# pangenome/povu

Measured on AMD Instinct MI355X. Metric: edges/sec decomposed (flubble+PVST), higher is better.
Workload: dtype u32

## Files before the change

include/povu_hip.h:

```cpp
#ifndef POVU_HIP_H
#define POVU_HIP_H

#include <stddef.h>
#include <stdint.h>

#ifdef __cplusplus
extern "C" {
#endif

#define POVU_HIP_NIL 0xFFFFFFFFu
#define POVU_SIDE_L 0
#define POVU_SIDE_R 1
#define POVU_TIP_NONE 0
#define POVU_TIP_L 1
#define POVU_TIP_R 2

typedef struct povu_hip_ctx povu_hip_ctx;
typedef struct povu_hip_forest povu_hip_forest;

int povu_hip_device_count(void);

povu_hip_ctx *povu_hip_create(int device, char *err, size_t errlen);
void povu_hip_destroy(povu_hip_ctx *ctx);
int povu_hip_release_workspace(povu_hip_ctx *ctx);
// ... 320 lines not shown
char *povu_hip_pvst_format(uint32_t n_pvst, const uint32_t *a_id, const uint32_t *z_id, const uint8_t *a_or,
			   const uint8_t *z_or, const uint32_t *parent, size_t *len);
char *povu_hip_pvst_format_fam(uint32_t n_pvst, const uint32_t *a_id, const uint32_t *z_id, const uint8_t *a_or,
			       const uint8_t *z_or, const uint32_t *parent, const uint8_t *fam, size_t *len);
void povu_hip_buffer_free(void *p);

typedef struct {
	uint32_t n;
	char *type;
	uint32_t *file_id;
	uint32_t *a_id, *z_id;
	uint8_t *a_or, *z_or;
	uint8_t *route;
	uint32_t *parent;
	uint32_t *height;
} povu_pvst_doc;
povu_pvst_doc *povu_pvst_parse(const char *text, size_t len, char *err, size_t errlen);

int povu_hip_gfa_write(const char *path, uint32_t n_vtx, const uint32_t *vid, uint32_t n_links, const uint32_t *v1,
		       const uint8_t *s1, const uint32_t *v2, const uint8_t *s2, char *err, size_t errlen);
void povu_pvst_doc_free(povu_pvst_doc *doc);

typedef struct {
	povu_hip_call_refs refs;
	uint32_t n_paths;
	const uint32_t *slot_of_path;
	const char *const *sample;
} povu_hip_call_names;
povu_hip_call_names *povu_hip_call_names_make(uint32_t n_paths, const char *const *path_name, uint32_t n_prefixes,
					      const char *const *prefix, char *err, size_t errlen);
void povu_hip_call_names_free(povu_hip_call_names *n);
int povu_hip_sites_add_tree(povu_hip_sites *s, uint32_t tree, uint32_t n, const uint32_t *id1, const uint32_t *id2,
			    const uint8_t *or1, const uint8_t *or2, const uint32_t *parent, const uint8_t *family);
povu_hip_sites *povu_hip_sites_of_docs(const povu_pvst_doc *const *docs, uint32_t n);
povu_hip_sites *povu_hip_forest_sites(const povu_hip_forest *f);
void povu_hip_sites_free(povu_hip_sites *s);
char *povu_hip_calls_vcf(const povu_hip_calls *c, const povu_hip_sites *sites, const povu_hip_call_names *names,
			 const char *const *path_name, const char *date, const char *only_prefix, uint32_t threads, size_t *len);
char *povu_hip_calls_vcf_profile(const povu_hip_calls *c, const povu_hip_sites *sites, const povu_hip_call_names *names,
				 const char *const *path_name, const char *date, const char *only_prefix, uint32_t threads, uint32_t profile,
				 size_t *len);
char *povu_hip_calls_vcf_rest(const povu_hip_calls *c, const povu_hip_sites *sites, const povu_hip_call_names *names,
			      const char *const *path_name, const char *date, const char *const *prefix, uint32_t n_prefixes, uint32_t threads,
			      uint32_t profile, size_t *len);

typedef struct {
	char name[48];
	double ms;
	uint32_t launches;
} povu_hip_stage_time;
int povu_hip_last_stage_times(const povu_hip_ctx *ctx, povu_hip_stage_time *out, int max);
uint32_t povu_hip_last_seq_redo(const povu_hip_ctx *ctx);
int povu_hip_last_black_only_classes(const povu_hip_ctx *ctx);
int povu_hip_last_laminar_check_ran(const povu_hip_ctx *ctx);
int povu_hip_last_crossings(povu_hip_ctx *ctx, uint32_t out[2]);
uint64_t povu_hip_last_links_processed(const povu_hip_ctx *ctx);

int povu_hip_debug_components(povu_hip_ctx *ctx, uint32_t *comp_of, uint32_t *local_idx);
int povu_hip_debug_tree(povu_hip_ctx *ctx, uint32_t comp, uint32_t *n_tree, uint32_t *gid, uint8_t *typ,
			uint32_t *par, uint32_t *cls);
int povu_hip_debug_edge_ids(povu_hip_ctx *ctx, uint32_t comp, uint32_t *n_tree, uint32_t *tree_edge_id);
int povu_hip_debug_stack(povu_hip_ctx *ctx, uint32_t comp, uint32_t *n, uint32_t *tree_vtx, uint32_t *cls,
			 uint32_t *next_seen);

#define POVU_HIP_SCAN_SUM 0
#define POVU_HIP_SCAN_MAX 1
#define POVU_HIP_SCAN_U64 2
#define POVU_HIP_SCAN_U8 3
#define POVU_HIP_SCAN_DIFF 4
#define POVU_HIP_SCAN_XOR_PAIR 5
#define POVU_HIP_SCAN_XOR_U128 6
#define POVU_HIP_SCAN_IN_PLACE 0x100
#define POVU_HIP_SCAN_N_DEV 0x200
int povu_hip_debug_scan(povu_hip_ctx *ctx, int op, const uint32_t *in, uint32_t *out, size_t n, const uint32_t *in2,
			uint32_t *out2, size_t n2);
int povu_hip_debug_sort(povu_hip_ctx *ctx, const uint32_t *keys, const uint32_t *vals, size_t n, unsigned bits,
			uint32_t *keys_out, uint32_t *vals_out);
int povu_hip_debug_compact(povu_hip_ctx *ctx, const uint8_t *flags, size_t n, uint32_t *out, uint32_t *count);
int povu_hip_debug_totals(povu_hip_ctx *ctx, const uint32_t *a, const uint32_t *b, size_t n, uint64_t tot[2]);
#define POVU_HIP_SEG_MIN 0
#define POVU_HIP_SEG_FIRST_LESS 1
#define POVU_HIP_SEG_LAST_LESS 2
int povu_hip_debug_segtree(povu_hip_ctx *ctx, const uint32_t *val, size_t n, const uint32_t *queries, size_t nq, uint32_t *out,
			   uint32_t *tree, uint32_t *P);
int povu_hip_debug_bitrank(povu_hip_ctx *ctx, const uint8_t *flags, size_t n, const uint32_t *pos, size_t nq, uint32_t *rank,
			   uint32_t *test, uint32_t *records);
int povu_hip_debug_append(povu_hip_ctx *ctx, const uint8_t *flags, size_t n, uint32_t *list, uint32_t *count);
int povu_hip_debug_list_rank(povu_hip_ctx *ctx, uint32_t n, const uint32_t *next, const uint8_t *w, const uint32_t *heads,
			     uint32_t nh, int mode, uint32_t bits, uint32_t *ra, uint32_t *rb);
double povu_hip_debug_scan_time(povu_hip_ctx *ctx, size_t n, int reps, int op);

uint64_t povu_hip_workspace_estimate(uint32_t n_vtx, uint32_t n_links, uint32_t n_components);
int povu_hip_workspace_breakdown(uint32_t n_vtx, uint32_t n_links, uint32_t n_components, uint64_t out[7]);
int povu_hip_prewarm(povu_hip_ctx *ctx, uint32_t n_vtx, uint32_t n_links, char *err, size_t errlen);
uint64_t povu_hip_leaf_workspace_estimate(uint32_t n_vtx, uint32_t n_components);

const char *povu_hip_version(void);

#ifdef __cplusplus
}
#endif
#endif
```

povu_amd/csrc/hip/common.hpp:

```cpp
#pragma once
#include <hip/hip_runtime.h>

#include <algorithm>
#include <cstdint>
#include <cstdio>
#include <cstring>
#include <stdexcept>
#include <string>
#include <vector>

#define POVU_NIL 0xFFFFFFFFu

__device__ __forceinline__ uint4 load4_unaligned(const unsigned *__restrict__ p)
{
	typedef unsigned v4a __attribute__((ext_vector_type(4), aligned(4)));
	const v4a v = *reinterpret_cast<const v4a *>(p);
	return make_uint4(v.x, v.y, v.z, v.w);
}

#ifdef POVU_XCD_SWIZZLE
__device__ __forceinline__ unsigned povu_xcd_bid()
{
	const unsigned nwg = gridDim.x, q = nwg >> 3, r = nwg & 7u, x = blockIdx.x & 7u, i = blockIdx.x >> 3;
	return (x < r ? x * (q + 1) : r * (q + 1) + (x - r) * q) + i;
// ... 220 lines not shown
		hipEvent_t a, b;
		uint32_t launches;
	};
	std::vector<Rec> recs;
	std::vector<hipEvent_t> pool;
	size_t pool_used = 0;
	hipStream_t stream = nullptr;
	bool enabled = true;
	hipEvent_t get()
	{
		if (pool_used == pool.size()) {
			hipEvent_t e;
			HIP_CHECK(hipEventCreate(&e));
			pool.push_back(e);
		}
		return pool[pool_used++];
	}
	void reset()
	{
		recs.clear();
		pool_used = 0;
	}
	void begin(const char *name)
	{
		if (!enabled)
			return;
		Rec r{name, get(), get(), 0};
		HIP_CHECK(hipEventRecord(r.a, stream));
		recs.push_back(r);
	}
	void end(uint32_t launches)
	{
		if (!enabled)
			return;
		recs.back().launches = launches;
		HIP_CHECK(hipEventRecord(recs.back().b, stream));
	}
	~StageTimer()
	{
		for (auto e : pool)
			(void)hipEventDestroy(e);
	}
};

void scan_exclusive_u32(const uint32_t *in, uint32_t *out, size_t n, void *tmp, size_t tmp_bytes, hipStream_t s);
void scan_exclusive_u32_pair(const uint32_t *in0, uint32_t *out0, size_t n0, const uint32_t *in1, uint32_t *out1, size_t n1,
			     void *tmp, size_t tmp_bytes, hipStream_t s);
void scan_exclusive_xor_u32_pair(const uint32_t *in0, uint32_t *out0, const uint32_t *in1, uint32_t *out1, size_t n, void *tmp,
				 size_t tmp_bytes, hipStream_t s);
void scan_exclusive_u8(const uint8_t *in0, uint32_t *out0, size_t n0, const uint8_t *in1, uint32_t *out1, size_t n1, void *tmp,
		       size_t tmp_bytes, hipStream_t s);
void scan_exclusive_diff_u32(const uint32_t *in, const uint32_t *sub, uint32_t *out, size_t n, void *tmp, size_t tmp_bytes,
			     hipStream_t s);
void scan_exclusive_xor_u128(const ulonglong2 *in, ulonglong2 *out, size_t n, void *tmp, size_t tmp_bytes, hipStream_t s,
			     const uint32_t *n_dev = nullptr);
size_t scan_tmp_bytes(size_t n);
void scan_exclusive_u64(const uint64_t *in, uint64_t *out, size_t n, uint64_t *tmp, hipStream_t s);
size_t scan_exclusive_u64_tmp(size_t n);
__device__ __forceinline__ uint32_t bitrank(const uint4 *__restrict__ rec, uint32_t x)
{
	const uint4 r = rec[x >> 6];
	const unsigned long long bits = (unsigned long long)r.x | ((unsigned long long)r.y << 32);
	return r.z + (uint32_t)__popcll(bits & ((1ull << (x & 63u)) - 1ull));
}
__device__ __forceinline__ bool bitrank_test(const uint4 *__restrict__ rec, uint32_t x)
{
	const uint4 r = rec[x >> 6];
	return (((x & 32u) ? r.y : r.x) >> (x & 31u)) & 1u;
}
struct StackComp {
	const uint4 *rec;
	const uint32_t *list;
	__device__ __forceinline__ uint32_t operator()(uint32_t i) const { return list[bitrank(rec, i + 1) - 1u]; }
};
__device__ __forceinline__ unsigned long long spread4(unsigned long long x)
{
	x &= 0xFFFFull;
	x = (x | (x << 24)) & 0x000000FF000000FFull;
	x = (x | (x << 12)) & 0x000F000F000F000Full;
	x = (x | (x << 6)) & 0x0303030303030303ull;
	x = (x | (x << 3)) & 0x1111111111111111ull;
	return x;
}
__device__ __forceinline__ void bitrank_store_wave(uint4 *__restrict__ rec, uint32_t f, bool in_range)
{
	const uint32_t lane = threadIdx.x & 63u;
	const unsigned long long m0 = __ballot(f & 1u), m1 = __ballot(f & 2u), m2 = __ballot(f & 4u), m3 = __ballot(f & 8u);
	if (lane < 4 && in_range) {
		const unsigned sh = 16u * lane;
		const unsigned long long w = spread4(m0 >> sh) | (spread4(m1 >> sh) << 1) | (spread4(m2 >> sh) << 2) | (spread4(m3 >> sh) << 3);
		rec[lane] = make_uint4((uint32_t)w, (uint32_t)(w >> 32), 0u, 0u);
	}
}
void bitrank_build(uint4 *rec, size_t n_rec, uint32_t *tmp_counts, void *scan_tmp, size_t scan_tmp_bytes, hipStream_t s);

static constexpr uint32_t LIST_ITER = 16, LIST_TPB = 256, LIST_SPAN = LIST_TPB * 4 * LIST_ITER;
__device__ __forceinline__ void append_in_order(unsigned long long fw, uint32_t B0, uint32_t *__restrict__ list, uint32_t *__restrict__ n_list)
{
	__shared__ uint32_t tot[LIST_ITER * (LIST_TPB / 64)], base_sh;
	const uint32_t lane = threadIdx.x & 63u, wave = threadIdx.x >> 6;
	const unsigned long long lt = (1ull << lane) - 1ull;
#pragma unroll
	for (uint32_t it = 0; it < LIST_ITER; it++) {
		const uint32_t f = (uint32_t)(fw >> (4 * it)) & 15u;
		const uint32_t t = (uint32_t)(__popcll(__ballot(f & 1u)) + __popcll(__ballot(f & 2u)) + __popcll(__ballot(f & 4u)) + __popcll(__ballot(f & 8u)));
		if (lane == 0)
// ... 54 lines not shown
```

povu_amd/csrc/hip/context.hpp:

```cpp
#pragma once
#include "../../../include/povu_hip.h"

#include "forest_wire.hpp"
#include "graph_kernels.hpp"
#include "leaf_kernels.hpp"
#include "par_kernels.hpp"
#include "seq_kernels.hpp"
#include "sub_kernels.hpp"
#include "tree_kernels.hpp"

#include <map>
#include <memory>
#include <mutex>
#include <numeric>
#include <string>

using namespace povu_hip;

struct PinnedPool {
	struct Block {
		void *p;
		size_t cap;
		int seg;
	};
// ... 144 lines not shown
		if (!q) {
			b.pool = pool;
			b.p = pool->get(block_bytes_for(total) + meta_bytes(meta_reserve), b.cap, &b.seg);
		}
		b.bytes = layout(b.p, total, &b);
		blocks.push_back(std::move(b));
		return blocks.back();
	}
	void release_blocks()
	{
		for (auto &b : blocks)
			if (b.p && b.pool)
				b.pool->put(b.p, b.cap, b.seg);
		blocks.clear();
	}
	~povu_hip_forest()
	{
		std::call_once(ready_once, [this] { wait_arrays(); });
		if (ev0)
			(void)hipEventDestroy(ev0);
		if (ev1)
			(void)hipEventDestroy(ev1);
		for (hipEvent_t e : more_events)
			(void)hipEventDestroy(e);
		release_blocks();
		if (xblk && pool)
			pool->put(xblk, xblk_cap, xblk_seg);
	}
	struct Tree : forest_wire::TreeRecord {
		int blk = 0;
	};
	std::vector<Tree> trees;
	std::vector<uint64_t> hairpins;
	void *xblk = nullptr;
	size_t xblk_cap = 0;
	int xblk_seg = -1;
	const void *walk_ctx = nullptr;
	uint64_t walk_gen = 0;
};

struct PassPlan {
	uint32_t rank = 0, world = 1;
	bool hairpins = false, all_seq = false, seq_tree = false, par_tree = true, leaf_sub = false, all_sub = false;
	bool sorted_adj = false, force_redo = false, redo_odd = false;
	bool big_class_dfs = false, sparse_splitters = false, all_vertex_classes = false, check_laminar = false;
	bool timed = true, overlap_tail = false, heaviest_first = false;
};

struct LastPass {
	bool valid = false;
	PassPlan plan;
	uint32_t C = 0, seq_redo = 0;
	bool mixed = false, redo_pvst_only = false, stack_export_pending = false;
};

struct povu_hip_ctx {
	int device = 0;
	hipStream_t stream = nullptr;
	SideStream side;
	ResidentGraph g;
	Arena ws_sub;
	size_t ws_sub_hint = 0;
	Arena ws, ws_b, ws2, ws_seq, ws_leaf, ws_walk, upload_tmp;
	HostScratch host;
	std::shared_ptr<PinnedPool> pool = std::make_shared<PinnedPool>();
	StageTimer timer;
	std::vector<povu_hip_stage_time> last_times;
	uint64_t last_links = 0;
	CompState cs{};
	SeqWs sw{};
	ParWs pw{};
	TreeWs tw{};
	LastPass last;
	std::vector<uint32_t> shard_comp_ids;
	uint32_t shard_total_components = 0;
	Arena shard_buf;
	Arena graph_arena;
	hipEvent_t tail_done = nullptr;
	SideStream walk_side;
	bool tail_pending = false;
	void wait_tail()
	{
		if (tail_pending) {
			(void)hipEventSynchronize(tail_done);
			tail_pending = false;
		}
	}
	void quiesce()
	{
		if (tail_pending) {
			(void)hipStreamSynchronize(stream);
			wait_tail();
		}
	}
	Arena wk_ws, wk_out;
	Arena paths_buf;
	uint32_t *path_steps = nullptr;
	uint64_t *path_off = nullptr;
	uint32_t n_paths = 0;
	uint64_t n_path_steps = 0, paths_gen = 0;
	bool paths_valid = false;
	Arena tr_ws, tr_task, tr_trav, tr_steps;
	Arena seq_buf, cl_ws, cl_slot, cl_rec, cl_spell, cl_bytes;
	Arena iv_ws, iv_heads, iv_rows;
	Arena nm_ws;
	Arena pr_ws, pr_slab, pr_rows;
// ... 67 lines not shown
```

povu_amd/csrc/hip/debug_hooks.hip:

```cpp
#include "context.hpp"
#include "segtree.hpp"

#include <algorithm>
#include <numeric>

using namespace povu_hip;

namespace
{
constexpr size_t DBG_GUARD = 256;
constexpr int DBG_GUARD_BYTE = 0xC5, DBG_POISON_BYTE = 0xA7;
constexpr int DBG_RC_GUARD = 5;
struct DbgOut {
	size_t bytes = 0;
	int fill = DBG_GUARD_BYTE;
	bool on = true;
	char *base = nullptr;
	size_t span = 0;
	template <class T>
	T *data() const { return reinterpret_cast<T *>(base + DBG_GUARD); }
	void declare(Spans &take, hipStream_t s)
	{
		if (!on)
			return;
// ... 12 lines not shown
	{
		take(bytes, p);
		if (take.ar && bytes)
			HIP_CHECK(hipMemsetAsync(p, DBG_POISON_BYTE, bytes, s));
	}
};
template <class T>
struct DbgIn {
	const T *host = nullptr;
	size_t n = 0;
	bool on = true;
	const T *dev = nullptr;
	void declare(Spans &take, hipStream_t s)
	{
		T *d = nullptr;
		if (on)
			take(n + 16, d);
		if (take.ar && on && n)
			HIP_CHECK(copy_async(d, host, n * sizeof(T), hipMemcpyHostToDevice, s));
		dev = d;
	}
};
template <class... B>
void dbg_carve(Arena &ar, hipStream_t s, B &...buf)
{
	carve(ar, [&](Spans &take) { (buf.declare(take, s), ...); });
}
bool dbg_all_guard(const void *host, size_t from, size_t to)
{
	const unsigned char *p = static_cast<const unsigned char *>(host);
	for (size_t i = from; i < to; i++)
		if (p[i] != (unsigned char)DBG_GUARD_BYTE)
			return false;
	return true;
}
bool dbg_guards_intact(const DbgOut &o, hipStream_t s)
{
	if (!o.base)
		return true;
	const size_t back = o.span - DBG_GUARD - o.bytes;
	std::vector<unsigned char> h(DBG_GUARD + back);
	HIP_CHECK(copy_async(h.data(), o.base, DBG_GUARD, hipMemcpyDeviceToHost, s));
	HIP_CHECK(copy_async(h.data() + DBG_GUARD, o.base + DBG_GUARD + o.bytes, back, hipMemcpyDeviceToHost, s));
	HIP_CHECK(hipStreamSynchronize(s));
	return dbg_all_guard(h.data(), 0, h.size());
}
}

extern "C" int povu_hip_debug_scan(povu_hip_ctx *ctx, int op, const uint32_t *in, uint32_t *out, size_t n, const uint32_t *in2,
				   uint32_t *out2, size_t n2)
{
	const int kind = op & 0xFF;
	const bool in_place = (op & POVU_HIP_SCAN_IN_PLACE) != 0, with_len = (op & POVU_HIP_SCAN_N_DEV) != 0;
	if (!ctx || kind > POVU_HIP_SCAN_XOR_U128 || (op & ~(0xFF | POVU_HIP_SCAN_IN_PLACE | POVU_HIP_SCAN_N_DEV)))
		return 1;
	if (kind == POVU_HIP_SCAN_U8) {
		if ((n && (!in || !out)) || (in2 && n2 && !out2))
			return 1;
	} else if (!in || !out || (in2 && !out2 && kind != POVU_HIP_SCAN_DIFF)) {
		return 1;
	}
	if ((in_place && (kind > POVU_HIP_SCAN_U64 || in2)) || (with_len && kind != POVU_HIP_SCAN_XOR_U128) ||
	    ((kind == POVU_HIP_SCAN_DIFF || kind == POVU_HIP_SCAN_XOR_PAIR) && !in2))
		return 1;
	try {
		HIP_CHECK(hipSetDevice(ctx->device));
		hipStream_t s = ctx->stream;
		const size_t e_in = kind == POVU_HIP_SCAN_U8 ? 1 : kind == POVU_HIP_SCAN_U64 ? 8 : kind == POVU_HIP_SCAN_XOR_U128 ? 16 : 4;
		const size_t e_out = kind == POVU_HIP_SCAN_U64 ? 8 : kind == POVU_HIP_SCAN_XOR_U128 ? 16 : 4;
		const bool pair = in2 && (kind == POVU_HIP_SCAN_SUM || kind == POVU_HIP_SCAN_U8 || kind == POVU_HIP_SCAN_XOR_PAIR);
		const bool second_in = pair || kind == POVU_HIP_SCAN_DIFF;
		const size_t m = !second_in ? 0 : (kind == POVU_HIP_SCAN_SUM || kind == POVU_HIP_SCAN_U8) ? n2 : n;
		const size_t tb = kind == POVU_HIP_SCAN_U64 ? scan_exclusive_u64_tmp(n) * 8 : scan_tmp_bytes(std::max(n, m));
		const uint32_t len = (uint32_t)n2;
		Arena ar;
		DbgOut o1{n * e_out}, o2{m * e_out, DBG_GUARD_BYTE, pair};
		DbgScratch scr{tb};
		DbgIn<char> i1{reinterpret_cast<const char *>(in), n * e_in, !in_place}, i2{reinterpret_cast<const char *>(in2), m * e_in, second_in};
		DbgIn<uint32_t> ilen{&len, 1, with_len};
		dbg_carve(ar, s, o1, o2, scr, i1, i2, ilen);
		if (in_place)
			HIP_CHECK(copy_async(o1.data<char>(), in, n * e_in, hipMemcpyHostToDevice, s));
		if (with_len)
			HIP_CHECK(hipStreamSynchronize(s));
		const char *di = in_place ? o1.data<char>() : i1.dev, *di2 = i2.dev;
		const uint32_t *w1 = reinterpret_cast<const uint32_t *>(di), *w2 = reinterpret_cast<const uint32_t *>(di2);
		void *tmp = scr.p;
		switch (kind) {
		case POVU_HIP_SCAN_SUM:
			if (pair)
				scan_exclusive_u32_pair(w1, o1.data<uint32_t>(), n, w2, o2.data<uint32_t>(), m, tmp, tb, s);
			else
				scan_exclusive_u32(w1, o1.data<uint32_t>(), n, tmp, tb, s);
			break;
		case POVU_HIP_SCAN_MAX: scan_exclusive_max_u32(w1, o1.data<uint32_t>(), n, tmp, tb, s); break;
		case POVU_HIP_SCAN_U64:
			scan_exclusive_u64(reinterpret_cast<const uint64_t *>(di), o1.data<uint64_t>(), n, static_cast<uint64_t *>(tmp), s);
			break;
		case POVU_HIP_SCAN_U8:
			scan_exclusive_u8(reinterpret_cast<const uint8_t *>(di), o1.data<uint32_t>(), n,
					  pair ? reinterpret_cast<const uint8_t *>(di2) : nullptr, pair ? o2.data<uint32_t>() : nullptr, m, tmp, tb, s);
			break;
		case POVU_HIP_SCAN_DIFF: scan_exclusive_diff_u32(w1, w2, o1.data<uint32_t>(), n, tmp, tb, s); break;
		case POVU_HIP_SCAN_XOR_PAIR: scan_exclusive_xor_u32_pair(w1, o1.data<uint32_t>(), w2, o2.data<uint32_t>(), n, tmp, tb, s); break;
		default:
			scan_exclusive_xor_u128(reinterpret_cast<const ulonglong2 *>(di), o1.data<ulonglong2>(), n, tmp, tb, s, ilen.dev);
			break;
		}
		if (n)
			HIP_CHECK(copy_async(out, o1.data<char>(), n * e_out, hipMemcpyDeviceToHost, s));
		if (pair && m)
			HIP_CHECK(copy_async(out2, o2.data<char>(), m * e_out, hipMemcpyDeviceToHost, s));
		HIP_CHECK(hipStreamSynchronize(s));
		if (!dbg_guards_intact(o1, s) || !dbg_guards_intact(o2, s))
			return DBG_RC_GUARD;
		if (with_len && !dbg_all_guard(out, std::min<size_t>(n2 + 1, n) * 16, n * 16))
			return DBG_RC_GUARD;
		return 0;
	} catch (const std::exception &) {
		return 2;
	}
}

extern "C" int povu_hip_debug_sort(povu_hip_ctx *ctx, const uint32_t *keys, const uint32_t *vals, size_t n, unsigned bits,
				   uint32_t *keys_out, uint32_t *vals_out)
{
	if (!ctx || bits > 32 || (n && (!keys || !vals || !keys_out || !vals_out)))
		return 1;
	try {
		HIP_CHECK(hipSetDevice(ctx->device));
		hipStream_t s = ctx->stream;
		const size_t tb = sort_tmp_bytes(n);
		Arena ar;
		DbgOut ko{n * 4}, vo{n * 4};
		DbgScratch tmp{tb};
		DbgIn<uint32_t> dk{keys, n}, dv{vals, n};
		dbg_carve(ar, s, ko, vo, tmp, dk, dv);
		sort_pairs_u32(dk.dev, ko.data<uint32_t>(), dv.dev, vo.data<uint32_t>(), n, bits, tmp.p, tb, s);
		if (n) {
			HIP_CHECK(copy_async(keys_out, ko.data<char>(), n * 4, hipMemcpyDeviceToHost, s));
			HIP_CHECK(copy_async(vals_out, vo.data<char>(), n * 4, hipMemcpyDeviceToHost, s));
		}
		HIP_CHECK(hipStreamSynchronize(s));
		return dbg_guards_intact(ko, s) && dbg_guards_intact(vo, s) ? 0 : DBG_RC_GUARD;
	} catch (const std::exception &) {
		return 2;
	}
}

extern "C" int povu_hip_debug_compact(povu_hip_ctx *ctx, const uint8_t *flags, size_t n, uint32_t *out, uint32_t *count)
{
	if (!ctx || !count || n >= (size_t(1) << 32) || (n && (!flags || !out)))
		return 1;
	try {
		HIP_CHECK(hipSetDevice(ctx->device));
		hipStream_t s = ctx->stream;
// ... 383 lines not shown
```

povu_amd/csrc/hip/par_kernels.hip:

```cpp
#include "par_kernels.hpp"
#include "segtree.hpp"

#include <algorithm>
#include <cstdlib>

namespace povu_hip
{

#define NIL POVU_NIL
static constexpr int TPB = 256;
static constexpr size_t PVST_STAGE_MIN = size_t(1) << 20;
static inline unsigned nblk(size_t n) { return (unsigned)((n + TPB - 1) / TPB); }
#define LAUNCH(k, n, s, ...)                                                                     \
	do {                                                                                     \
		if ((n) > 0) {                                                                   \
			hipLaunchKernelGGL(k, dim3(nblk(n)), dim3(TPB), 0, s, __VA_ARGS__);      \
			HIP_CHECK(hipGetLastError());                                            \
		}                                                                                \
	} while (0)

__global__ void k_tcomp_vertices(uint32_t V, uint32_t T, const uint32_t *__restrict__ ckey, const uint32_t *__restrict__ voff,
				 uint32_t *__restrict__ t_comp)
{
	uint32_t i = BIDX * blockDim.x + threadIdx.x;
	if (i >= V)
		return;
	uint32_t c = ckey[i];
	t_comp[2 * i + c] = c;
	t_comp[2 * i + 1 + c] = c;
	if (i + 1 == voff[c + 1])
		t_comp[2 * i + 2 + c] = c;
	if (i == V - 1)
		t_comp[T] = NIL;
}
__global__ void k_globalize(uint32_t T, const uint32_t *__restrict__ t_comp, const uint32_t *__restrict__ voff,
			    const uint32_t *__restrict__ c_ntree, const uint32_t *__restrict__ t_par,
			    const uint32_t *__restrict__ t_size, uint32_t *__restrict__ gpar, uint32_t *__restrict__ gsize,
			    uint32_t *__restrict__ t_root, uint32_t *__restrict__ hi0, uint32_t *__restrict__ cov,
			    const uint32_t *__restrict__ depth, uint32_t *__restrict__ mpre, uint32_t *__restrict__ incnt,
			    uint32_t *__restrict__ srccnt)
{
	uint32_t t = BIDX * blockDim.x + threadIdx.x;
	if (t >= T)
		return;
	srccnt[t] = 0;
	if (t == T - 1)
		srccnt[T] = srccnt[T + 1] = 0;
	if (cov) {
		hi0[t] = NIL;
		cov[t] = 0;
		incnt[t] = 0;
		if (t == T - 1) {
			hi0[T] = NIL;
			cov[T] = 0;
			incnt[T] = incnt[T + 1] = 0;
		}
	} else if (t == T - 1) {
		hi0[T] = NIL;
	}
	uint32_t c = t_comp[t];
	uint32_t base = 2 * voff[c] + c, l = t - base, n = c_ntree[c];
	t_root[t] = base;
	if (l < n) {
		uint32_t p = t_par[t], sz = t_size[t];
		gpar[t] = p == NIL ? NIL : base + p;
		gsize[t] = sz;
		mpre[t] = base + depth[t] + n - l - sz;
	} else {
		gpar[t] = NIL;
		gsize[t] = 0;
		mpre[t] = NIL;
	}
}
__global__ void k_dense_be(uint32_t NB0, uint32_t C, const uint32_t *__restrict__ dbo, const uint32_t *__restrict__ voff,
			   const uint32_t *__restrict__ eoff, const uint32_t *__restrict__ be_src,
			   const uint32_t *__restrict__ be_tgt, uint32_t *__restrict__ b_src, uint32_t *__restrict__ b_tgt)
{
	uint32_t j = BIDX * blockDim.x + threadIdx.x;
	if (j >= NB0)
		return;
	uint32_t lo = 0, hi = C;
	while (hi - lo > 1) {
		uint32_t mid = (lo + hi) >> 1;
		if (dbo[mid] <= j)
			lo = mid;
		else
			hi = mid;
	}
	uint32_t c = lo, b = j - dbo[c];
	uint64_t tb = 2ull * voff[c] + c, bb = (uint64_t)eoff[c] + voff[c] + 2 * tb;
	b_src[j] = (uint32_t)tb + be_src[bb + b];
	b_tgt[j] = (uint32_t)tb + be_tgt[bb + b];
}

__global__ void k_hi0(uint32_t NB0, const uint32_t *__restrict__ b_src, const uint32_t *__restrict__ b_tgt,
		      uint32_t *__restrict__ hi0, uint32_t *__restrict__ cov, uint32_t *__restrict__ incnt)
{
	uint32_t j = BIDX * blockDim.x + threadIdx.x;
	if (j >= NB0)
		return;
// ... 134 lines not shown
				simp[t] = (uint8_t)sm;
				if (t == T - 1)
					simp[T] = 0;
				if (hpf)
					hpf[t] = (uint8_t)sm;
				capf[t] = 0;
				b4 |= bch << (t - t0);
			}
		}
		bw |= (unsigned long long)b4 << (4 * it);
	}
	append_in_order(bw, B0, br_list, n_br);
}
__global__ void k_capping(const uint32_t *__restrict__ n_list, const uint32_t *__restrict__ list, const uint32_t *__restrict__ gsize,
			  const uint32_t *__restrict__ hi0, const uint4 *__restrict__ brec, const RootOf root_of, const SegTree segA,
			  uint32_t *__restrict__ cap_tgt, uint8_t *__restrict__ capf, uint32_t *__restrict__ literal_rule_seen)
{
	const uint32_t n = *n_list;
	for (uint32_t i = BIDX * blockDim.x + threadIdx.x; i < n; i += gridDim.x * blockDim.x)
		capping_of(list[i], gsize, hi0, brec, root_of, segA, cap_tgt, capf, literal_rule_seen);
}
static constexpr uint32_t BX_TILE = TPB;
__global__ void __launch_bounds__(TPB) k_flag_tile_counts(uint32_t T, const uint8_t *__restrict__ capf, const uint8_t *__restrict__ simp,
							   uint32_t *__restrict__ tcap, uint32_t *__restrict__ tsimp, uint32_t ntiles)
{
	const uint32_t e0 = (blockIdx.x * TPB + threadIdx.x) * 16u;
	uint32_t nc = 0, ns = 0;
	if (e0 + 16 <= T) {
		const uint4 a = *reinterpret_cast<const uint4 *>(capf + e0), b = *reinterpret_cast<const uint4 *>(simp + e0);
		const uint32_t wa[4] = {a.x, a.y, a.z, a.w}, wb[4] = {b.x, b.y, b.z, b.w};
#pragma unroll
		for (int k = 0; k < 4; k++)
#pragma unroll
			for (int q = 0; q < 4; q++) {
				nc += ((wa[k] >> (8 * q)) & 0xFFu) ? 1u : 0u;
				ns += ((wb[k] >> (8 * q)) & 0xFFu) ? 1u : 0u;
			}
	} else {
		for (uint32_t k = e0; k < T; k++) {
			nc += capf[k] ? 1u : 0u;
			ns += simp[k] ? 1u : 0u;
		}
	}
	for (int off = 8; off; off >>= 1) {
		nc += __shfl_down(nc, off, 16);
		ns += __shfl_down(ns, off, 16);
	}
	const uint32_t tile = (blockIdx.x * TPB + threadIdx.x) / 16u;
	if ((threadIdx.x & 15u) == 0 && tile <= ntiles) {
		tcap[tile] = tile < ntiles ? nc : 0u;
		tsimp[tile] = tile < ntiles ? ns : 0u;
	}
}
__global__ void __launch_bounds__(TPB) k_bracket_extra(uint32_t T, uint32_t NB0_host, const uint32_t *__restrict__ nb0_dev, uint32_t ntiles,
							uint32_t nb_cap, const uint8_t *__restrict__ capf,
							const uint32_t *__restrict__ tcap, const uint8_t *__restrict__ simp,
							const uint32_t *__restrict__ tsimp, const uint32_t *__restrict__ cap_tgt,
							const RootOf root_of, uint32_t *__restrict__ b_src, uint32_t *__restrict__ b_tgt,
							const uint32_t *__restrict__ ordcnt, const uint32_t *__restrict__ gsize,
							const uint32_t *__restrict__ mpre, uint32_t *__restrict__ incnt,
							uint32_t *__restrict__ srccnt)
{
	const uint32_t NB0 = nb0_dev ? *nb0_dev : NB0_host, ncap = tcap[ntiles];
	if ((uint64_t)NB0 + ncap + tsimp[ntiles] > nb_cap)
		return;
	const uint32_t v0 = (BIDX * blockDim.x + threadIdx.x) * 4u, lane = threadIdx.x & 63u, tile = v0 / BX_TILE;
	uint32_t cw = 0, sw = 0;
	if (v0 + 4 <= T) {
		cw = *reinterpret_cast<const uint32_t *>(capf + v0);
		sw = *reinterpret_cast<const uint32_t *>(simp + v0);
	} else {
		for (uint32_t j = 0; v0 + j < T && j < 4; j++) {
			cw |= (capf[v0 + j] ? 1u : 0u) << (8 * j);
			sw |= (simp[v0 + j] ? 1u : 0u) << (8 * j);
		}
	}
	const unsigned long long lt = (1ull << lane) - 1ull;
	uint32_t rc = 0, rs = 0;
#pragma unroll
	for (int j = 0; j < 4; j++) {
		rc += (uint32_t)__popcll(__ballot(((cw >> (8 * j)) & 0xFFu) != 0) & lt);
		rs += (uint32_t)__popcll(__ballot(((sw >> (8 * j)) & 0xFFu) != 0) & lt);
	}
	if (v0 >= T)
		return;
	if (cw)
		rc += tcap[tile];
	if (sw)
		rs += tsimp[tile];
	uint4 oc = make_uint4(0u, 0u, 0u, 0u), gs = oc, mp = oc;
	if (ordcnt) {
		if (v0 + 4 <= T) {
			oc = *reinterpret_cast<const uint4 *>(ordcnt + v0);
			gs = *reinterpret_cast<const uint4 *>(gsize + v0);
			mp = *reinterpret_cast<const uint4 *>(mpre + v0);
		} else {
			uint32_t *o = &oc.x, *g = &gs.x, *m = &mp.x;
			for (uint32_t j = 0; v0 + j < T && j < 4; j++)
				o[j] = ordcnt[v0 + j], g[j] = gsize[v0 + j], m[j] = mpre[v0 + j];
		}
	}
	const uint32_t ocv[4] = {oc.x, oc.y, oc.z, oc.w}, gsv[4] = {gs.x, gs.y, gs.z, gs.w}, mpv[4] = {mp.x, mp.y, mp.z, mp.w};
#pragma unroll
	for (uint32_t j = 0; j < 4; j++) {
		const uint32_t v = v0 + j;
		if (v >= T)
			break;
		const uint32_t c = (cw >> (8 * j)) & 0xFFu, sm = (sw >> (8 * j)) & 0xFFu;
		if (c) {
			const uint32_t q = NB0 + rc++;
			const uint32_t tg = cap_tgt[v];
			b_src[q] = v;
			b_tgt[q] = tg;
			if (ordcnt)
				atomicAdd(&incnt[tg], 1u);
		}
		if (sm) {
			const uint32_t q = NB0 + ncap + rs++;
			const uint32_t root = root_of(v);
			b_src[q] = v;
			b_tgt[q] = root;
			if (ordcnt)
				atomicAdd(&incnt[root], 1u);
		}
		if (ordcnt && gsv[j])
			srccnt[mpv[j]] = ocv[j] + (c ? 1u : 0u) + (sm ? 1u : 0u);
	}
}
__global__ void k_bracket_order(uint32_t NB, uint32_t NB0, uint32_t ncap, uint32_t nsimp, const uint32_t *__restrict__ b_src,
				const uint32_t *__restrict__ b_tgt, const uint32_t *__restrict__ mpre,
				uint32_t *__restrict__ key, uint32_t *__restrict__ val, uint32_t *__restrict__ incnt,
				uint32_t *__restrict__ srccnt)
{
	uint32_t q = BIDX * blockDim.x + threadIdx.x;
	if (q >= NB)
		return;
	uint32_t j;
	if (q < nsimp)
		j = NB0 + ncap + q;
	else if (q < nsimp + ncap)
		j = NB0 + (q - nsimp);
	else
		j = NB0 - 1 - (q - nsimp - ncap);
	uint32_t m = mpre[b_src[j]];
	key[q] = m;
	val[q] = j;
	atomicAdd(&incnt[b_tgt[j]], 1u);
	atomicAdd(&srccnt[m], 1u);
}
__global__ void k_bracket_place(uint32_t NB, uint32_t NB0, uint32_t ncap, const uint32_t *__restrict__ b_src,
				const uint32_t *__restrict__ b_tgt, const uint32_t *__restrict__ b_ord,
				const uint32_t *__restrict__ mpre, const uint32_t *__restrict__ bstart,
				const uint8_t *__restrict__ capf, const uint8_t *__restrict__ simp,
				uint32_t *__restrict__ tgtR, uint32_t *__restrict__ rid)
{
	uint32_t j = BIDX * blockDim.x + threadIdx.x;
	if (j >= NB)
		return;
	const uint32_t v = b_src[j];
	uint32_t rank;
	if (j < NB0)
		rank = bstart[mpre[v] + 1] - bstart[mpre[v]] - 1 - b_ord[j];
	else if (j < NB0 + ncap)
		rank = simp[v];
	else
		rank = 0;
	const uint32_t pos = bstart[mpre[v]] + rank;
	tgtR[pos] = b_tgt[j];
	if (rid)
		rid[pos] = j;
}
__global__ void k_gather_u32(uint32_t n, const uint32_t *__restrict__ idx, const uint32_t *__restrict__ src,
			     uint32_t *__restrict__ dst)
{
	uint32_t i = BIDX * blockDim.x + threadIdx.x;
	if (i < n)
		dst[i] = src[idx[i]];
}
struct StackPlace {
// ... 556 lines not shown
{
	uint32_t c = BIDX * blockDim.x + threadIdx.x;
	if (c >= T)
		return;
	const uint32_t ci = t_comp[c];
	if (ci == NIL)
		return;
	const uint32_t base = t_root[c], end = base + c_ntree[ci];
	if (c == base && c_ntree[ci])
		c_nbry[ci] = ps[end] - ps[base];
	if (!push[c])
		return;
	const uint32_t after = ps[end] - ps[c + 1];
	const uint64_t pb = (uint64_t)voff[ci] + ci;
	out[2 * (pb + after)] = b12[2 * (size_t)c];
	out[2 * (pb + after) + 1] = b12[2 * (size_t)c + 1];
}

void run_parallel_hairpins(const CompState &cs, SeqWs &sw, ParWs &pw, uint32_t C, StageTimer &tm, hipStream_t s)
{
	const uint32_t T = 2 * sw.V + C;
	tm.begin("par_hairpins");
	LAUNCH(k_hp_inputs, T, s, T, pw.gsize, pw.gpar, pw.hpf, pw.hp1, pw.hp2, pw.hp3);
	seg_build(pw.segH1, pw.hp1, T, s);
	seg_build(pw.segH2, pw.hp2, T, s);
	seg_build(pw.segH3, pw.hp3, T, s);
	uint8_t *push = pw.f8a;
	uint32_t *pps = pw.psA;
	unsigned long long *b12 = pw.hp_b12;
	if (!b12 || !pw.hpf || !pw.t_comp)
		throw HipError("hairpin report: its arrays were not carved (internal)");
	LAUNCH(k_hp_close, T, s, T, pw.gsize, pw.t_root, pw.t_comp, sw.c_ntree, sw.t_gid, pw.hp3, pw.segH1, pw.segH2, pw.segH3, push,
	       b12);
	scan_exclusive_u8(push, pps, (size_t)T + 1, nullptr, nullptr, 0, pw.scan_tmp, pw.scan_tmp_bytes, s);
	LAUNCH(k_hp_emit, T, s, T, push, pps, pw.t_root, pw.t_comp, sw.c_ntree, cs.voff, b12, (unsigned long long *)sw.hairpins,
	       sw.c_nbry);
	tm.end(10);
}

static void for_each_span(ParWs &pw, size_t V, size_t E, size_t Cmax, int groups, const StageWsOpts &o, Spans &spans)
{
	auto take1 = [&](size_t n, auto *&...p) {
		if (groups & 1)
			spans(n, p...);
	};
	auto take = [&](size_t n, auto *&...p) {
		if (groups & 2)
			spans(n, p...);
	};
	const size_t T = 2 * V + Cmax, NB = o.nb_cap ? std::min(o.nb_cap, E + V + T) : E + V + T, S = V + 1;
	pw.nb_cap = NB;
	auto skip = [](auto **p) { *p = nullptr; };
	take1(T + 2, pw.hi0, pw.mpre, pw.dlt, pw.incnt, pw.lsz);
	take1(NB + 2, pw.b_src, pw.b_tgt, pw.b_ord);
	take1(V + 4, pw.sdl);
	take1(16, pw.err);
	take1(Cmax + 2, pw.comp_bad);
	pw.scan_tmp_bytes = std::max(scan_tmp_bytes(std::max(T, NB) + 4), 2 * compact_tmp_bytes(std::max(T, NB) + 4));
	pw.sort_tmp_bytes = sort_tmp_bytes(std::max(std::max(T, NB), std::max(4 * V, 2 * E) + 8) + 4);
	take1(pw.scan_tmp_bytes, pw.scan_tmp);
	take1(pw.sort_tmp_bytes, pw.sort_tmp);
	for (uint32_t **p : {&pw.t_comp, &pw.t_root, &pw.gpar, &pw.gsize, &pw.cov}) {
		if (o.full_t)
			take(T + 2, *p);
		else if (groups & 2)
			skip(p);
	}
	take(T + 2, pw.psA, pw.psB, pw.flagC, pw.psC, pw.cap_tgt, pw.dlt_ps, pw.psin, pw.topi, pw.gcls, pw.vals_t, pw.vals_t2);
	take(T + 32, pw.f8a, pw.f8b, pw.f8c, pw.f8d);
	take(T + 2, pw.keys_t, pw.keys_t2);
	take(Cmax + 2, pw.dbo);
	take(NB + 2, pw.b_val2, pw.tgtR);
	for (uint32_t **p : {&pw.b_val, &pw.b_key, &pw.b_key2}) {
		if (o.sorted_brackets)
			take(NB + 2, *p);
		else if (groups & 2)
			skip(p);
	}
	take(S + 2, pw.s_vtx, pw.s_cls, pw.ns, pw.prev, pw.lev, pw.e_i);
	take(S / 64 + 3, pw.erec, pw.crec);
	take(S / 64 + 3, pw.rk_cnt);
	take(Cmax + 2, pw.clist);
	take(S + 4, pw.walk, pw.walk_ps, pw.wrun);
	take(Cmax + 2, pw.cproc_ps, pw.doff);
	take(SegTree::tree_words(T + 1), pw.segA.tree);
	take(SegTree::tree_words(NB + 1), pw.segB.tree);
	take(SegTree::tree_words(S + 1), pw.segP.tree, pw.segL.tree);
	take(((S + Cmax + 2) * 4 + 64) * 3 + ((S + Cmax + 2) + 64) * 2 + 256, pw.stage);
	if (o.hairpins) {
		take(2 * T + 4, pw.hp_b12);
		take(T + 2, pw.hpf);
		take(T + 2, pw.hp1, pw.hp2, pw.hp3);
		take(SegTree::tree_words(T + 1), pw.segH1.tree, pw.segH2.tree, pw.segH3.tree);
	} else if (groups & 2) {
		pw.hpf = nullptr;
		pw.hp_b12 = nullptr;
		pw.hp1 = pw.hp2 = pw.hp3 = nullptr;
		pw.segH1.tree = pw.segH2.tree = pw.segH3.tree = nullptr;
	}
}

size_t par_workspace_bytes(size_t V, size_t E, size_t Cmax, int groups, const StageWsOpts &o)
{
	ParWs tmp{};
	return measure([&](Spans &take) { for_each_span(tmp, V, E, Cmax, groups, o, take); }) + (1 << 20);
}
// ... 7 lines not shown
__global__ void k_summary(uint32_t C, const uint32_t *__restrict__ err, const uint32_t *__restrict__ bad,
			  const uint32_t *__restrict__ status, const uint32_t *__restrict__ npvst,
			  const uint32_t *__restrict__ nbry, const uint32_t *__restrict__ doff, uint32_t *__restrict__ out)
{
	uint32_t i = BIDX * blockDim.x + threadIdx.x;
	if (i > C)
		return;
	if (i == 0) {
		out[0] = err ? err[0] : 0;
		out[1] = err ? (err[1] | (err[8] << 1)) : 0;
		out[2] = err ? err[2] : 0;
		out[3] = err ? err[3] : 0;
	}
	uint32_t *o = out + 4;
	if (i < C) {
		o[i] = bad ? bad[i] : 0;
		o[(size_t)C + i] = status[i];
		o[2 * (size_t)C + i] = npvst[i];
		o[3 * (size_t)C + i] = nbry[i];
	}
	o[4 * (size_t)C + i] = doff ? doff[i] : 0;
}

void pass_summary(const SeqWs &sw, const ParWs *pw, uint32_t C, uint32_t *host_out, hipStream_t s)
{
	uint32_t *dev_out = nullptr;
	HIP_CHECK(hipHostGetDevicePointer(reinterpret_cast<void **>(&dev_out), host_out, 0));
	LAUNCH(k_summary, (size_t)C + 1, s, C, pw ? pw->err : nullptr, pw ? pw->comp_bad : nullptr, sw.c_status, sw.c_npvst,
	       sw.c_nbry, pw ? pw->doff : nullptr, dev_out);
}

void run_parallel_dg(const CompState &cs, SeqWs &sw, ParWs &pw, uint32_t C, uint32_t n_processed, uint32_t n_stack,
		     int64_t dense_nb0, const std::function<void *(size_t)> &alloc_result_block, StageTimer &tm, hipStream_t s,
		     const SideStream &side, PassTail &tail)
{
	const uint32_t V = sw.V, T = 2 * V + C;
	const bool want_hp = sw.hairpins != nullptr;
	pw.V = V;
	pw.E = sw.E;
	pw.C = C;
	pw.T = T;
	auto scan = [&](const uint32_t *in, uint32_t *out, size_t n) {
		scan_exclusive_u32(in, out, n, pw.scan_tmp, pw.scan_tmp_bytes, s);
	};
	auto scan8 = [&](const uint8_t *in, uint32_t *out, size_t n) {
		scan_exclusive_u8(in, out, n, nullptr, nullptr, 0, pw.scan_tmp, pw.scan_tmp_bytes, s);
	};
	auto scan2 = [&](const uint32_t *in0, uint32_t *out0, size_t n0, const uint32_t *in1, uint32_t *out1, size_t n1) {
		scan_exclusive_u32_pair(in0, out0, n0, in1, out1, n1, pw.scan_tmp, pw.scan_tmp_bytes, s);
	};

	tm.begin("par_setup");
	const bool lean = dense_nb0 >= 0 && !want_hp;
	if (lean) {
		pw.gsize = sw.t_size;
		pw.gpar = sw.t_par;
	} else {
		LAUNCH(k_tcomp_vertices, V, s, V, T, cs.ckey, cs.voff, pw.t_comp);
		LAUNCH(k_globalize, T, s, T, pw.t_comp, cs.voff, sw.c_ntree, sw.t_par, sw.t_size, pw.gpar, pw.gsize, pw.t_root, pw.hi0,
		       dense_nb0 >= 0 ? nullptr : pw.cov, sw.t_depth, pw.mpre, pw.incnt, pw.dlt);
	}
	const RootOf root_of{lean ? nullptr : pw.t_root, cs.voff, C};
	uint32_t NB0;
	if (dense_nb0 >= 0) {
		NB0 = dense_nb0 == NB0_ON_DEVICE ? 0u : (uint32_t)dense_nb0;
	} else {
		scan(sw.c_nbe0, pw.dbo, (size_t)C + 1);
		NB0 = pw.host->read_u32(pw.dbo + C, s);
		LAUNCH(k_dense_be, NB0, s, NB0, C, pw.dbo, cs.voff, cs.eoff, sw.be_src, sw.be_tgt, pw.b_src, pw.b_tgt);
	}
	tm.end(7);

	tm.begin("par_classes");
	if (dense_nb0 < 0)
		LAUNCH(k_hi0, NB0, s, NB0, pw.b_src, pw.b_tgt, pw.hi0, pw.cov, nullptr);
	seg_build(pw.segA, pw.hi0, T, s);
	uint8_t *simp = pw.f8b, *capf = pw.f8c;
	uint32_t *pssimp = pw.psB, *pscap = pw.psC;
	uint4 *brec = reinterpret_cast<uint4 *>(pw.psA);
	uint32_t *brec_cnt = reinterpret_cast<uint32_t *>(pw.f8a);
	uint32_t *pscov = pw.psB;
	if (dense_nb0 >= 0)
		scan_exclusive_diff_u32(pw.lsz, pw.incnt, pscov, (size_t)T + 1, pw.scan_tmp, pw.scan_tmp_bytes, s);
	else
		scan(pw.cov, pscov, (size_t)T + 1);
	KLAUNCH(k_bridge_flags, dim3(nblk(((size_t)T / 256 + 1) * 64)), dim3(TPB), 0, s, T, pw.gsize, pw.gpar, pscov, brec);
	bitrank_build(brec, (size_t)T / 64 + 1, brec_cnt, pw.scan_tmp, pw.scan_tmp_bytes, s);
	uint32_t *br_list = pw.vals_t, *n_br = pw.err + 10;
	KLAUNCH(k_hi_simp, dim3((unsigned)(((size_t)T + HS_VERTS - 1) / HS_VERTS)), dim3(TPB), 0, s, T, pw.gsize, brec, simp, want_hp ? pw.hpf : nullptr, capf, br_list,
		n_br);
	KLAUNCH(k_capping, dim3(std::min<unsigned>(nblk(T / 8 + 1), 16384)), dim3(TPB), 0, s, n_br, br_list, pw.gsize, pw.hi0, brec, root_of,
		pw.segA, pw.cap_tgt, capf, pw.err + 5);
	const uint32_t ntiles = (T + BX_TILE - 1) / BX_TILE;
	uint32_t *tsimp = pssimp, *tcap = pscap;
	KLAUNCH(k_flag_tile_counts, dim3((ntiles + 1 + 15) / 16 + 1), dim3(TPB), 0, s, T, capf, simp, tcap, tsimp, ntiles);
	scan_exclusive_u32_pair(tsimp, tsimp, (size_t)ntiles + 1, tcap, tcap, (size_t)ntiles + 1, pw.scan_tmp, pw.scan_tmp_bytes, s);
	uint32_t *srccnt = pw.dlt, *bstart = pw.dlt_ps;
	uint32_t *extra = pw.host->take<uint32_t>(4);
	publish_words(extra, WordSrc{{tcap + ntiles, tsimp + ntiles, pw.err + 5, pw.err + 6}}, 4, s);
	const HostScratch::Token extra_ready = pw.host->mark(s);
	LAUNCH(k_bracket_extra, ((size_t)T + 3) / 4, s, T, NB0, dense_nb0 == NB0_ON_DEVICE ? pw.err + 6 : nullptr, ntiles,
	       (uint32_t)std::min<size_t>(pw.nb_cap, 0xFFFFFFFFu), capf, tcap, simp, tsimp, pw.cap_tgt, root_of, pw.b_src, pw.b_tgt,
	       dense_nb0 >= 0 ? pw.lsz : nullptr, pw.gsize, pw.mpre, pw.incnt, srccnt);
	if (dense_nb0 >= 0)
		scan2(pw.incnt, pw.psin, (size_t)T + 1, srccnt, bstart, (size_t)T + 1);
	pw.host->wait(extra_ready);
	if (dense_nb0 == NB0_ON_DEVICE) {
		NB0 = extra[3];
		if (NB0 > pw.nb_cap)
			throw HipError("spanning tree: more back edges than links outside the tree and sides without links (internal sizing bug)");
	}
	const uint32_t ncap = extra[0], nsimp = extra[1], NB = NB0 + ncap + nsimp;
	pw.nb0 = NB0;
	pw.ncap = ncap;
	pw.nsimp = nsimp;
	if ((size_t)NB > pw.nb_cap)
		throw HipError("class stage: more brackets than the workspace was sized for (internal sizing bug)");
	if (dense_nb0 < 0 && !pw.b_key)
		throw HipError("class stage: the bracket sort's buffers were not carved for a sequential tree stage (internal)");
	if (!lean && !pw.t_comp)
		throw HipError("class stage: the per-vertex tables were not carved (internal)");
	const bool black_only = !want_hp && !pw.all_vertex_classes && extra[2] == 0;
	pw.black_only_used = black_only;
	if (dense_nb0 >= 0) {
		LAUNCH(k_bracket_place, NB, s, NB, NB0, ncap, pw.b_src, pw.b_tgt, pw.b_ord, pw.mpre, bstart, capf, simp, pw.tgtR,
		       want_hp ? pw.b_val2 : nullptr);
	} else {
		uint32_t *bk = pw.b_key, *bk2 = pw.b_key2;
		LAUNCH(k_bracket_order, NB, s, NB, NB0, ncap, nsimp, pw.b_src, pw.b_tgt, pw.mpre, bk, pw.b_val, pw.incnt, srccnt);
		scan2(pw.incnt, pw.psin, (size_t)T + 1, srccnt, bstart, (size_t)T + 1);
		sort_pairs_u32(bk, bk2, pw.b_val, pw.b_val2, NB, bits_for(T), pw.sort_tmp, pw.sort_tmp_bytes, s);
		LAUNCH(k_gather_u32, NB, s, NB, pw.b_val2, pw.b_tgt, pw.tgtR);
	}
	seg_build(pw.segB, pw.tgtR, NB, s);
	uint32_t *ck = pw.keys_t, *ck2 = pw.keys_t2;
	const uint32_t NC = black_only ? V : T;
	const uint32_t S = n_stack;
	uint8_t *cflag = pw.f8a;
	uint32_t *cps = pw.psA;
	uint8_t *dflag = pw.f8c;
	if (black_only) {
		uint32_t *sdl = pw.dlt;
		if (pw.sdl_filled && dense_nb0 >= 0) {
			sdl = pw.sdl;
		} else {
			HIP_CHECK(hipMemsetAsync(pw.dlt, 0, ((size_t)V + 2) * 4, s));
			LAUNCH(k_shift_delta, V, s, V, cs.ckey, sw.c_ntree, pw.gsize, pw.dlt);
		}
		uint32_t *shift_ps = pw.topi;
		scan(sdl, shift_ps, (size_t)V + 1);
		const StackPlace sp{cs.voff, pw.soff, sdl, shift_ps, pw.s_vtx};
		LAUNCH(k_top_bracket<true>, NC, s, NC, pw.gsize, pw.gpar, pw.mpre, bstart, pw.segB, pw.tgtR, pw.psin, ck,
		       pw.vals_t, pw.lsz, pw.err, pw.b_val2, NB0 + ncap, nullptr, cs.ckey, sw.c_ntree, sp);
		sort_pairs_u32(ck, ck2, pw.vals_t, pw.vals_t2, NC, bits_for((uint64_t)NB + 1), pw.sort_tmp, pw.sort_tmp_bytes, s);
		tm.end(30 + 2 * 22);
		tm.begin("par_stack");
		LAUNCH(k_class_finish_black, std::max<size_t>(((size_t)NC + 3) / 4, 1), s, NC, S, ck2, pw.vals_t2, pw.lsz, cflag, pw.ns, pw.prev,
// ... 167 lines not shown
```

povu_amd/csrc/hip/par_kernels.hpp:

```cpp
#pragma once
#include "common.hpp"
#include "graph_kernels.hpp"
#include "seq_kernels.hpp"

#include <functional>

namespace povu_hip
{

struct SegTree {
	uint32_t *tree = nullptr;
	const uint32_t *val = nullptr;
	uint32_t P = 1;
	static constexpr uint32_t BLK = 16;
	static uint32_t pow2(size_t n)
	{
		uint32_t p = 1;
		while (p < n)
			p <<= 1;
		return p;
	}
	static size_t tree_words(size_t n) { return 2 * (size_t)pow2((n + BLK - 1) / BLK + 1); }
};

struct ParWs {
	HostScratch *host;
	uint32_t V, E, C, T;
	bool all_vertex_classes = false;
	bool check_laminar = false;
	bool laminar_checked = false;
	bool black_only_used = false;
	bool s_cls_valid = false;
	bool gcls_valid = false;
	uint32_t *t_comp, *t_root, *gpar, *gsize;
	uint32_t *hi0, *cov, *psA, *psB, *flagC, *psC;
	uint8_t *f8a, *f8b, *f8c, *f8d;
	uint32_t *cap_tgt, *mpre, *dlt, *dlt_ps, *incnt, *psin, *topi, *lsz, *gcls;
	uint32_t *sdl;
	bool sdl_filled = false;
	uint32_t *vals_t, *vals_t2;
	uint32_t *keys_t, *keys_t2;
	uint32_t *dbo;
	uint32_t *b_src, *b_tgt, *b_val, *b_val2, *tgtR, *b_ord;
	uint32_t *b_key, *b_key2;
	size_t nb_cap = 0;
	uint32_t *s_vtx, *s_cls, *ns, *prev;
	uint32_t *soff;
	uint32_t *walk, *walk_ps, *wrun;
	uint32_t *lev, *e_i;
	uint4 *erec, *crec;
	uint32_t *clist, *rk_cnt;
	StackComp stack_comp() const { return StackComp{crec, clist}; }
	uint32_t *comp_bad;
	uint32_t *cproc_ps, *doff;
	size_t d_total;
	uint32_t n_stack;
	uint32_t nb0 = 0, ncap = 0, nsimp = 0;
	uint32_t n_emitted = 0;
	uint32_t *d_a, *d_z, *d_parent;
	uint8_t *d_aor, *d_zor;
	void *stage;
	uint32_t *err;
	SegTree segA, segB, segP, segL;
	uint8_t *hpf;
	uint32_t *hp1, *hp2, *hp3;
	unsigned long long *hp_b12;
	SegTree segH1, segH2, segH3;
	void *scan_tmp, *sort_tmp;
	size_t scan_tmp_bytes, sort_tmp_bytes;
};

struct SideStream {
	hipStream_t stream = nullptr;
	hipEvent_t fork = nullptr, join = nullptr;
	hipEvent_t fork2 = nullptr;
};

struct PassTail {
	bool want_overlap = false;
	hipEvent_t done = nullptr;
	hipEvent_t done2 = nullptr;
	const uint32_t *early_summary = nullptr;
	bool summary_final = false;
	bool overlapped = false;
};

struct StageWsOpts {
	size_t nb_cap = 0;
	bool full_t = true;
	bool sorted_brackets = true;
// ... 20 lines not shown
```

povu_amd/csrc/hip/povu_hip.hip:

```cpp
#include "context.hpp"

#include <algorithm>
#include <atomic>
#include <cstdlib>
#include <memory>
#include <mutex>
#include <numeric>

#include <fcntl.h>
#include <sys/mman.h>
#include <unistd.h>

using namespace povu_hip;

PinnedPool::~PinnedPool()
{
	for (auto &b : free_blocks)
		if (b.seg < 0)
			(void)hipHostFree(b.p);
	for (auto &sg : segments) {
		(void)hipHostUnregister(sg.p);
		(void)munmap(sg.p, sg.cap);
		(void)shm_unlink(segment_name(shared_tag, sg.seg).c_str());
	}
// ... 738 lines not shown
	bool carved = false;
	void carve()
	{
		if (carved)
			return;
		ctx->wait_tail();
		ctx->ws_seq.reserve(carve_workspace(nullptr, 2, z, ctx->cs, ctx->sw, hairpins));
		carve_workspace(&ctx->ws_seq, 2, z, ctx->cs, ctx->sw, hairpins);
		carved = true;
	}
	void init(hipStream_t s)
	{
		carve();
		const SeqWs &sw = ctx->sw;
		for (uint32_t *p : {sw.first_child, sw.o_head, sw.i_head, sw.bl, sw.t_hi, sw.t_cls, sw.st_head, sw.st_tail})
			HIP_CHECK(hipMemsetAsync(p, 0xFF, z.T * 4, s));
		HIP_CHECK(hipMemsetAsync(sw.ctr, 0xFF, z.nS * 4, s));
		HIP_CHECK(hipMemsetAsync(sw.cur, 0, z.nS * 4, s));
		HIP_CHECK(hipMemsetAsync(sw.selfloop, 0, z.V, s));
		HIP_CHECK(hipMemsetAsync(sw.last, 0xFF, (z.B + z.T) * 4, s));
		HIP_CHECK(hipMemsetAsync(sw.in_s, 0, z.B + z.T, s));
	}
};

struct RowsOut {
	const uint32_t *sum = nullptr;
	uint32_t nbad = 0;
	bool mixed = false;
	bool redo_pvst_only = false, stack_export_pending = false;
	bool fast_tail = false;
	PassTail tail;
};

static const uint32_t *read_summary(povu_hip_ctx *ctx, uint32_t C, bool with_par, const povu_hip_forest &f)
{
	uint32_t *h = ctx->host.take<uint32_t>(5 * (size_t)C + 8);
	count_kernel_d2h((5 * (size_t)C + 8) * 4);
	pass_summary(ctx->sw, with_par ? &ctx->pw : nullptr, C, h, ctx->stream);
	HIP_CHECK(hipEventRecord(f.ev1, ctx->stream));
	HIP_CHECK(hipStreamSynchronize(ctx->stream));
	return h;
}

static int64_t parallel_rows(povu_hip_ctx *ctx, const PassPlan &p, uint32_t C, const uint32_t *gstats, const CompTables &t,
			     povu_hip_forest &f, SeqLanes &lanes, StageTimer &tm, RowsOut &out)
{
	SeqWs &sw = ctx->sw;
	ParWs &pw = ctx->pw;
	hipStream_t s = ctx->stream;
	int64_t dense_nb0 = -1;
	pw.cproc_ps = sw.tables + 2 * ((size_t)C + 1);
	ctx->tw.cproc = sw.tables + 3 * ((size_t)C + 1);
	pw.soff = sw.tables + 4 * ((size_t)C + 1);
	if (p.seq_tree) {
		lanes.init(s);
		tm.begin("tree_seq");
		sw.stages = SEQ_STAGE_TREE;
		launch_seq_components(sw, s);
		tm.end(1);
	} else {
		dense_nb0 = run_parallel_tree(ctx->cs, sw, pw, ctx->tw, C, t.event_lists, gstats[0], p.big_class_dfs, p.sparse_splitters, tm, s);
	}
	pw.all_vertex_classes = p.all_vertex_classes;
	pw.check_laminar = p.check_laminar;
	out.tail.want_overlap = p.overlap_tail;
	out.tail.done = f.ev1;
	out.tail.done2 = ctx->tail_done;
	auto alloc_result_block = [&f](size_t total) -> void * {
		f.release_blocks();
		void *dev = nullptr;
		HIP_CHECK(hipHostGetDevicePointer(&dev, f.alloc(total).p, 0));
		return dev;
	};
	run_parallel_dg(ctx->cs, sw, pw, C, t.n_processed, t.n_stack, dense_nb0, alloc_result_block, tm, s, ctx->side, out.tail);
	out.stack_export_pending = true;
	if (p.redo_odd)
		mark_odd_u32(pw.comp_bad, C, s);
	out.fast_tail = out.tail.summary_final && !p.leaf_sub && !p.hairpins && !p.force_redo && !p.redo_odd;
	const uint32_t *sum = out.sum = out.fast_tail ? out.tail.early_summary : read_summary(ctx, C, true, f);
	if (sum[0])
		throw HipError("parallel class stage: a tree vertex has no live bracket (internal invariant broken)");
	if (sum[1] & 1u)
		throw HipError("list ranking: splitter capacity exceeded (internal sizing bug)");
	if (sum[1] & 2u)
		throw HipError("class walk: stack pool exhausted (internal sizing bug)");
	if (sum[2])
		throw HipError("spanning forest of the links has the wrong size (internal)");
	if (sum[3])
		throw HipError("candidate stack has the wrong size (internal)");
	for (uint32_t c = 0; c < C; c++)
		out.nbad += sum[4 + c] ? 1 : 0;
	return dense_nb0;
}

static void leaf_passes(povu_hip_ctx *ctx, const PassPlan &p, uint32_t C, uint32_t nbad, povu_hip_forest &f, LeafState &leaf_state,
			StageTimer &tm)
{
	hipStream_t s = ctx->stream;
	if (nbad && p.hairpins)
		throw HipError("leaf subflubble passes: with --hairpins a component that needs the sequential redo is rebuilt "
			       "from scratch by the one-lane kernels, whose tree state the passes do not read");
	tm.begin("leaf_subflubbles");
	leaf_prepare(ctx->cs, ctx->sw, ctx->pw, ctx->tw, C, ctx->ws_leaf, leaf_state, s);
	leaf_dense(leaf_state, ctx->sw, ctx->pw, C, s);
	const size_t n = ctx->pw.d_total;
	povu_hip_forest::Block &b = f.blocks.empty() ? f.alloc(n) : f.blocks[0];
	f.labels = n != 0;
	b.sub_ai.resize(n, ctx->pool);
	b.sub_zi.resize(n, ctx->pool);
	b.sub_fam.resize(n, ctx->pool);
	if (n) {
		HIP_CHECK(copy_async(b.sub_ai.data(), leaf_state.dense.ai, n * 4, hipMemcpyDeviceToHost, s));
		HIP_CHECK(copy_async(b.sub_zi.data(), leaf_state.dense.zi, n * 4, hipMemcpyDeviceToHost, s));
// ... 268 lines not shown

extern "C" povu_hip_forest *povu_hip_decompose(povu_hip_ctx *ctx, const povu_hip_opts *opts, char *err, size_t errlen)
{
	std::unique_ptr<povu_hip_forest> f;
	XferScope xfer(ctx);
	try {
		if (ctx && !ctx->g.block && ctx->shard_total_components) {
			f = std::make_unique<povu_hip_forest>();
			f->pool = ctx->pool;
			f->total_components = ctx->shard_total_components;
			ctx->last_times.clear();
			ctx->last_links = 0;
			return f.release();
		}
		if (!ctx || !ctx->g.block)
			throw HipError("no graph resident: call povu_hip_graph_upload first");
		HIP_CHECK(hipSetDevice(ctx->device));
		const PassPlan p = plan_pass(opts);
		if (!p.overlap_tail)
			ctx->wait_tail();
		const ResidentGraph &g = ctx->g;
		Sizes z{g.V, g.E, g.V, 0, 0, 2 * (size_t)g.V, g.n_slots};
		ctx->last = LastPass{};
		ctx->host.reset();
		ctx->cs.host = ctx->pw.host = ctx->tw.host = &ctx->host;
		reserve(ctx, ctx->ws, rowb_carve_label(nullptr, z, ctx->cs));
		rowb_carve_label(&ctx->ws, z, ctx->cs);
		StageTimer &tm = ctx->timer;
		tm.reset();
		tm.enabled = p.timed;
		f = std::make_unique<povu_hip_forest>();
		f->pool = ctx->pool;
		HIP_CHECK(hipEventCreate(&f->ev0));
		HIP_CHECK(hipEventCreate(&f->ev1));
		HIP_CHECK(hipEventRecord(f->ev0, ctx->stream));

		const RowB rb = row_b(ctx, p, z, tm);
		const uint32_t C = rb.C;
		z.set_components(C);
		const bool tail_waited = carve_stages(ctx, p, z, C, tm);
		ctx->host.wait(rb.sizes);
		const CompTables tables = component_tables(ctx, p, C, rb.voff, rb.eoff, tail_waited);
		f->meta_reserve = (size_t)C + 1;
		SeqLanes lanes{ctx, z, p.hairpins};
		LeafState leaf_state;
		RowsOut out = rows_c_to_g(ctx, p, C, rb.gstats, tables, *f, lanes, leaf_state, tm);
		fetch_result(ctx, p, C, rb.voff, rb.eoff, out, *f, leaf_state, tm);
		if (!p.leaf_sub)
			ctx->ws_leaf.release();
		if (!p.all_sub)
			ctx->ws_sub.release();
		stage_times(ctx, tm, *f);
		ctx->last = LastPass{true, p, C, out.nbad, out.mixed, out.redo_pvst_only, out.stack_export_pending};
		if (p.world == 1 && ctx->shard_comp_ids.empty()) {
			f->walk_ctx = ctx;
			f->walk_gen = g.gen;
		}
		return f.release();
	} catch (const std::exception &e) {
		if (ctx && ctx->stream)
			(void)hipStreamSynchronize(ctx->stream);
		if (ctx && ctx->side.stream)
			(void)hipStreamSynchronize(ctx->side.stream);
		f.reset();
		set_err(err, errlen, e.what());
		return nullptr;
	}
}

extern "C" uint32_t povu_hip_forest_total_components(const povu_hip_forest *f) { return f ? f->total_components : 0; }
extern "C" uint32_t povu_hip_forest_tree_count(const povu_hip_forest *f) { return f ? (uint32_t)f->trees.size() : 0; }

extern "C" int povu_hip_forest_wait(povu_hip_forest *f)
{
	if (!f)
		return 1;
	f->ready();
	return 0;
}
extern "C" double povu_hip_forest_pass_ms(povu_hip_forest *f)
{
	if (!f)
		return -1.0;
	f->ready();
	return f->pass_ms;
}

extern "C" double povu_hip_forest_span_ms(povu_hip_forest *first, povu_hip_forest *last)
{
	if (!first || !last || !first->ev0 || !last->ev1)
		return -1.0;
	first->ready();
	last->ready();
	float ms = 0;
	return hipEventElapsedTime(&ms, first->ev0, last->ev1) == hipSuccess ? (double)ms : -1.0;
}

extern "C" int povu_hip_forest_get(const povu_hip_forest *f, uint32_t i, povu_hip_tree *out)
{
	if (!f || !out || i >= f->trees.size())
		return 1;
	const_cast<povu_hip_forest *>(f)->ready();
	const auto &t = f->trees[i];
	out->component_id = t.component_id;
	out->n_vtx = t.n_vtx;
	out->n_links = t.n_links;
// ... 230 lines not shown
			e[-1] = (char)('0' + v);
	};
	memcpy(o, "H\t0.0.3\t.\t.\t.\n", 14);
	o += 14;
	for (uint32_t v = 0; v < n; v++) {
		*o++ = fam ? (char)fam[v] : (v == 0 ? 'D' : 'F');
		*o++ = '\t';
		put(v);
		*o++ = '\t';
		if (v == 0) {
			*o++ = '.';
		} else {
			*o++ = t.a_or[v] ? '<' : '>';
			put(t.a_id[v]);
			*o++ = t.z_or[v] ? '<' : '>';
			put(t.z_id[v]);
		}
		*o++ = '\t';
		const uint32_t c0 = coff[v], c1 = coff[v + 1];
		if (c0 == c1) {
			*o++ = '.';
		} else {
			for (uint32_t k = c0; k < c1; k++) {
				put(cadj[k]);
				if (k + 1 < c1)
					*o++ = ',', *o++ = ' ';
			}
		}
		*o++ = '\t';
		*o++ = v == 0 ? '.' : 'L';
		*o++ = '\n';
	}
	*o = 0;
	if (len)
		*len = (size_t)(o - buf);
	return buf;
}

extern "C" int povu_hip_last_stage_times(const povu_hip_ctx *ctx, povu_hip_stage_time *out, int max)
{
	if (!ctx)
		return 0;
	int n = (int)ctx->last_times.size();
	if (out)
		for (int i = 0; i < n && i < max; i++)
			out[i] = ctx->last_times[i];
	return n;
}

extern "C" uint32_t povu_hip_last_seq_redo(const povu_hip_ctx *ctx) { return ctx ? ctx->last.seq_redo : 0; }

extern "C" uint64_t povu_hip_last_links_processed(const povu_hip_ctx *ctx) { return ctx ? ctx->last_links : 0; }

extern "C" int povu_hip_last_black_only_classes(const povu_hip_ctx *ctx)
{
	return ctx && ctx->last.valid && !ctx->last.plan.all_seq && ctx->pw.black_only_used ? 1 : 0;
}

extern "C" int povu_hip_last_crossings(povu_hip_ctx *ctx, uint32_t out[2])
{
	if (!ctx || !out)
		return 1;
	out[0] = out[1] = 0;
	if (!ctx->last.valid || ctx->last.plan.all_seq || !ctx->pw.laminar_checked)
		return 0;
	ctx->quiesce();
	if (hipSetDevice(ctx->device) != hipSuccess)
		return 2;
	return hipMemcpy(out, ctx->pw.err + 11, 8, hipMemcpyDeviceToHost) == hipSuccess ? 0 : 2;
}

extern "C" int povu_hip_last_laminar_check_ran(const povu_hip_ctx *ctx)
{
	return ctx && ctx->last.valid && !ctx->last.plan.all_seq && ctx->pw.laminar_checked ? 1 : 0;
}
```

povu_amd/csrc/hip/primitives.hip:

```cpp
#include "common.hpp"

namespace povu_hip
{

static constexpr int SC_TPB = 256, SC_ITEMS = 8, SC_TILE = SC_TPB * SC_ITEMS, SC_MAX_BLOCKS = 1024;

template <int MAX>
__device__ __forceinline__ uint32_t sc_op(uint32_t a, uint32_t b)
{
	return MAX == 1 ? (a > b ? a : b) : (MAX == 2 ? (a ^ b) : a + b);
}
template <int MAX>
__device__ __forceinline__ uint32_t sc_block_reduce(uint32_t v, uint32_t *sh)
{
	for (int off = 32; off; off >>= 1)
		v = sc_op<MAX>(v, __shfl_down(v, off));
	if ((threadIdx.x & 63) == 0)
		sh[threadIdx.x >> 6] = v;
	__syncthreads();
	uint32_t r = sc_op<MAX>(sc_op<MAX>(sh[0], sh[1]), sc_op<MAX>(sh[2], sh[3]));
	__syncthreads();
	return r;
}
struct ScanJob {
	const uint32_t *in;
	const uint32_t *sub;
	const uint8_t *in8;
	uint32_t *out;
	size_t n, chunk;
	uint32_t blocks;
	uint32_t *partial;
	uint32_t tiles;
	unsigned long long *status;
	uint32_t *ticket;
};
struct ScanJobs {
	ScanJob j[2];
};
template <int MAX>
__global__ void __launch_bounds__(SC_TPB) k_scan_partials(const ScanJobs jobs)
{
	__shared__ uint32_t sh[4];
	const ScanJob &J = jobs.j[blockIdx.y];
	if (blockIdx.x >= J.blocks)
		return;
	const uint32_t *__restrict__ in = J.in;
	uint32_t *__restrict__ partial = J.partial;
	const size_t n = J.n, chunk = J.chunk;
	const size_t b0 = (size_t)blockIdx.x * chunk, b1 = b0 + chunk < n ? b0 + chunk : n;
	uint32_t acc = 0;
	auto fold4 = [&](const uint4 &a) { acc = sc_op<MAX>(acc, sc_op<MAX>(sc_op<MAX>(a.x, a.y), sc_op<MAX>(a.z, a.w))); };
	if (J.in8) {
		const uint8_t *__restrict__ in8 = J.in8;
		const size_t w1 = b0 + ((b1 - b0) & ~size_t(15));
		auto bytes4 = [](uint32_t w) {
			return sc_op<MAX>(sc_op<MAX>(w & 0xFFu, (w >> 8) & 0xFFu), sc_op<MAX>((w >> 16) & 0xFFu, w >> 24));
		};
		for (size_t i = b0 + 16 * (size_t)threadIdx.x; i < w1; i += 16 * SC_TPB) {
			const uint4 a = *reinterpret_cast<const uint4 *>(in8 + i);
			fold4(make_uint4(bytes4(a.x), bytes4(a.y), bytes4(a.z), bytes4(a.w)));
		}
		for (size_t i = w1 + threadIdx.x; i < b1; i += SC_TPB)
			acc = sc_op<MAX>(acc, in8[i]);
	} else {
		const uint32_t *__restrict__ sub = J.sub;
		const size_t w1 = b0 + ((b1 - b0) & ~size_t(3));
		if (sub) {
			for (size_t i = b0 + 4 * (size_t)threadIdx.x; i < w1; i += 4 * SC_TPB) {
				const uint4 a = *reinterpret_cast<const uint4 *>(in + i), c = *reinterpret_cast<const uint4 *>(sub + i);
				fold4(make_uint4(a.x - c.x, a.y - c.y, a.z - c.z, a.w - c.w));
			}
		} else {
			for (size_t i = b0 + 4 * (size_t)threadIdx.x; i < w1; i += 4 * SC_TPB)
				fold4(*reinterpret_cast<const uint4 *>(in + i));
		}
		for (size_t i = w1 + threadIdx.x; i < b1; i += SC_TPB)
			acc = sc_op<MAX>(acc, in[i] - (sub ? sub[i] : 0u));
	}
	acc = sc_block_reduce<MAX>(acc, sh);
	if (threadIdx.x == 0)
		partial[blockIdx.x] = acc;
}
__device__ __forceinline__ void sc_load_tile(const ScanJob &J, size_t e0, size_t b1, uint32_t (&v)[SC_ITEMS])
{
	if (J.in8) {
		const uint8_t *__restrict__ in8 = J.in8;
		if (e0 + SC_ITEMS <= b1) {
			const uint2 a = *reinterpret_cast<const uint2 *>(in8 + e0);
			v[0] = a.x & 0xFFu, v[1] = (a.x >> 8) & 0xFFu, v[2] = (a.x >> 16) & 0xFFu, v[3] = a.x >> 24;
			v[4] = a.y & 0xFFu, v[5] = (a.y >> 8) & 0xFFu, v[6] = (a.y >> 16) & 0xFFu, v[7] = a.y >> 24;
		} else {
			for (int k = 0; k < SC_ITEMS; k++)
				v[k] = e0 + k < b1 ? in8[e0 + k] : 0u;
		}
	} else if (e0 + SC_ITEMS <= b1) {
		const uint32_t *__restrict__ in = J.in;
		const uint4 a = *reinterpret_cast<const uint4 *>(in + e0), b = *reinterpret_cast<const uint4 *>(in + e0 + 4);
		v[0] = a.x, v[1] = a.y, v[2] = a.z, v[3] = a.w, v[4] = b.x, v[5] = b.y, v[6] = b.z, v[7] = b.w;
		if (J.sub) {
			const uint4 c = *reinterpret_cast<const uint4 *>(J.sub + e0), d = *reinterpret_cast<const uint4 *>(J.sub + e0 + 4);
			v[0] -= c.x, v[1] -= c.y, v[2] -= c.z, v[3] -= c.w, v[4] -= d.x, v[5] -= d.y, v[6] -= d.z, v[7] -= d.w;
		}
	} else {
		for (int k = 0; k < SC_ITEMS; k++)
			v[k] = e0 + k < b1 ? J.in[e0 + k] - (J.sub ? J.sub[e0 + k] : 0u) : 0u;
	}
}
template <int MAX>
__global__ void __launch_bounds__(SC_TPB) k_scan_chunks(const ScanJobs jobs)
{
	__shared__ uint32_t sh[4];
	__shared__ uint32_t wave_tot[4];
	const ScanJob &J = jobs.j[blockIdx.y];
	if (blockIdx.x >= J.blocks)
		return;
	uint32_t *__restrict__ out = J.out;
	const uint32_t *__restrict__ partial = J.partial;
	const size_t n = J.n, chunk = J.chunk;
	uint32_t base = 0;
	for (uint32_t k = threadIdx.x; k < blockIdx.x; k += SC_TPB)
		base = sc_op<MAX>(base, partial[k]);
	uint32_t carry = sc_block_reduce<MAX>(base, sh);
	const size_t b0 = (size_t)blockIdx.x * chunk, b1 = b0 + chunk < n ? b0 + chunk : n;
	const int lane = threadIdx.x & 63, wave = threadIdx.x >> 6;
	uint32_t v[SC_ITEMS], nx[SC_ITEMS];
	if (b0 < b1)
		sc_load_tile(J, b0 + (size_t)threadIdx.x * SC_ITEMS, b1, v);
	for (size_t t0 = b0; t0 < b1; t0 += SC_TILE) {
		const size_t e0 = t0 + (size_t)threadIdx.x * SC_ITEMS;
		const bool more = t0 + SC_TILE < b1;
		if (more)
			sc_load_tile(J, e0 + SC_TILE, b1, nx);
		uint32_t tot = 0;
		for (int k = 0; k < SC_ITEMS; k++) {
			const uint32_t x = v[k];
			v[k] = tot;
			tot = sc_op<MAX>(tot, x);
		}
		uint32_t inc = tot;
		for (int off = 1; off < 64; off <<= 1) {
			const uint32_t y = __shfl_up(inc, off);
			if (lane >= off)
				inc = sc_op<MAX>(inc, y);
		}
		if (lane == 63)
			wave_tot[wave] = inc;
// ... 25 lines not shown
}

static constexpr unsigned long long LB_AGG = 1ull << 32, LB_PREFIX = 2ull << 32;
template <int MAX, int LB_SUB, bool TICKET>
__global__ void __launch_bounds__(SC_TPB) k_scan_lookback(const ScanJobs jobs)
{
	constexpr int LB_TILE = SC_TILE * LB_SUB;
	__shared__ uint32_t wave_tot[LB_SUB][4];
	__shared__ uint32_t s_tile, s_carry;
	const ScanJob &J = jobs.j[blockIdx.y];
	if (blockIdx.x >= J.tiles)
		return;
	const int lane = threadIdx.x & 63, wave = threadIdx.x >> 6;
	uint32_t t = blockIdx.x;
	if (TICKET && J.tiles > 1) {
		if (threadIdx.x == 0)
			s_tile = atomicAdd(J.ticket, 1u);
		__syncthreads();
		t = s_tile;
	}
	const size_t b0 = (size_t)t * LB_TILE, b1 = b0 + LB_TILE < J.n ? b0 + LB_TILE : J.n;
	uint32_t v[LB_SUB][SC_ITEMS], inc[LB_SUB];
	if (b0 + LB_TILE <= J.n && !J.in8) {
		const uint32_t *__restrict__ in = J.in + b0 + (size_t)threadIdx.x * SC_ITEMS;
		uint4 a[LB_SUB][2];
#pragma unroll
		for (int q = 0; q < LB_SUB; q++)
			a[q][0] = *reinterpret_cast<const uint4 *>(in + q * SC_TILE), a[q][1] = *reinterpret_cast<const uint4 *>(in + q * SC_TILE + 4);
		if (J.sub) {
			const uint32_t *__restrict__ sub = J.sub + b0 + (size_t)threadIdx.x * SC_ITEMS;
#pragma unroll
			for (int q = 0; q < LB_SUB; q++) {
				const uint4 c = *reinterpret_cast<const uint4 *>(sub + q * SC_TILE), d = *reinterpret_cast<const uint4 *>(sub + q * SC_TILE + 4);
				a[q][0].x -= c.x, a[q][0].y -= c.y, a[q][0].z -= c.z, a[q][0].w -= c.w;
				a[q][1].x -= d.x, a[q][1].y -= d.y, a[q][1].z -= d.z, a[q][1].w -= d.w;
			}
		}
#pragma unroll
		for (int q = 0; q < LB_SUB; q++) {
			v[q][0] = a[q][0].x, v[q][1] = a[q][0].y, v[q][2] = a[q][0].z, v[q][3] = a[q][0].w;
			v[q][4] = a[q][1].x, v[q][5] = a[q][1].y, v[q][6] = a[q][1].z, v[q][7] = a[q][1].w;
		}
	} else if (b0 + LB_TILE <= J.n) {
		const uint8_t *__restrict__ in8 = J.in8 + b0 + (size_t)threadIdx.x * SC_ITEMS;
		uint2 a[LB_SUB];
#pragma unroll
		for (int q = 0; q < LB_SUB; q++)
			a[q] = *reinterpret_cast<const uint2 *>(in8 + q * SC_TILE);
#pragma unroll
		for (int q = 0; q < LB_SUB; q++) {
			v[q][0] = a[q].x & 0xFFu, v[q][1] = (a[q].x >> 8) & 0xFFu, v[q][2] = (a[q].x >> 16) & 0xFFu, v[q][3] = a[q].x >> 24;
			v[q][4] = a[q].y & 0xFFu, v[q][5] = (a[q].y >> 8) & 0xFFu, v[q][6] = (a[q].y >> 16) & 0xFFu, v[q][7] = a[q].y >> 24;
		}
	} else {
#pragma unroll
		for (int q = 0; q < LB_SUB; q++)
			sc_load_tile(J, b0 + (size_t)q * SC_TILE + (size_t)threadIdx.x * SC_ITEMS, b1, v[q]);
	}
#pragma unroll
	for (int q = 0; q < LB_SUB; q++) {
		uint32_t tot = 0;
#pragma unroll
		for (int k = 0; k < SC_ITEMS; k++) {
			const uint32_t x = v[q][k];
			v[q][k] = tot;
			tot = sc_op<MAX>(tot, x);
		}
		uint32_t i = tot;
		for (int off = 1; off < 64; off <<= 1) {
			const uint32_t y = __shfl_up(i, off);
			if (lane >= off)
				i = sc_op<MAX>(i, y);
		}
		inc[q] = i;
		if (lane == 63)
			wave_tot[q][wave] = i;
	}
	__syncthreads();
	if (wave == 0) {
		uint32_t agg = 0;
#pragma unroll
		for (int q = 0; q < LB_SUB; q++)
#pragma unroll
			for (int w = 0; w < 4; w++)
				agg = sc_op<MAX>(agg, wave_tot[q][w]);
		uint32_t carry = 0;
		if (t > 0) {
			if (lane == 0)
				__hip_atomic_store(J.status + t, LB_AGG | agg, __ATOMIC_RELAXED, __HIP_MEMORY_SCOPE_AGENT);
			for (int64_t base = (int64_t)t - 1;;) {
				const int64_t idx = base - lane;
				const unsigned long long w = idx >= 0 ? __hip_atomic_load(J.status + idx, __ATOMIC_RELAXED, __HIP_MEMORY_SCOPE_AGENT) : LB_PREFIX;
				const unsigned long long has_p = __ballot((w >> 32) == 2ull), unset = __ballot((w >> 32) == 0ull);
				const int stop = has_p ? __ffsll((long long)has_p) - 1 : 64;
				const unsigned long long need = stop >= 63 ? ~0ull : ((2ull << stop) - 1ull);
				if (unset & need)
					continue;
				uint32_t x = lane <= stop ? (uint32_t)w : 0u;
				for (int off = 32; off; off >>= 1)
					x = sc_op<MAX>(x, __shfl_down(x, off));
				carry = sc_op<MAX>(carry, __shfl(x, 0));
				if (has_p)
					break;
				base -= 64;
			}
		}
// ... 106 lines not shown
		return;
	if (tmp_bytes < SC_MAX_BLOCKS * sizeof(uint32_t))
		throw HipError("scan: temporary storage too small");
	ScanJobs jobs{};
	jobs.j[0] = make_scan_job(in, out, n, static_cast<uint32_t *>(tmp));
	if (scan_lookback<MAX>(jobs, 1, tmp, tmp_bytes, s))
		return;
	KLAUNCH(k_scan_partials<MAX>, dim3(jobs.j[0].blocks, 1), dim3(SC_TPB), 0, s, jobs);
	KLAUNCH(k_scan_chunks<MAX>, dim3(jobs.j[0].blocks, 1), dim3(SC_TPB), 0, s, jobs);
}

void scan_exclusive_u8(const uint8_t *in0, uint32_t *out0, size_t n0, const uint8_t *in1, uint32_t *out1, size_t n1, void *tmp,
		       size_t tmp_bytes, hipStream_t s)
{
	if (tmp_bytes < 2 * SC_MAX_BLOCKS * sizeof(uint32_t))
		throw HipError("scan: temporary storage too small");
	ScanJobs jobs{};
	unsigned gx = 0, gy = 0;
	if (n0) {
		jobs.j[gy] = make_scan_job(nullptr, out0, n0, static_cast<uint32_t *>(tmp) + gy * SC_MAX_BLOCKS, in0);
		gx = std::max(gx, jobs.j[gy].blocks);
		gy++;
	}
	if (in1 && n1) {
		jobs.j[gy] = make_scan_job(nullptr, out1, n1, static_cast<uint32_t *>(tmp) + gy * SC_MAX_BLOCKS, in1);
		gx = std::max(gx, jobs.j[gy].blocks);
		gy++;
	}
	if (!gy)
		return;
	if (scan_lookback<0>(jobs, (int)gy, tmp, tmp_bytes, s))
		return;
	KLAUNCH(k_scan_partials<0>, dim3(gx, gy), dim3(SC_TPB), 0, s, jobs);
	KLAUNCH(k_scan_chunks<0>, dim3(gx, gy), dim3(SC_TPB), 0, s, jobs);
}

void scan_exclusive_u32(const uint32_t *in, uint32_t *out, size_t n, void *tmp, size_t tmp_bytes, hipStream_t s)
{
	scan_exclusive<0>(in, out, n, tmp, tmp_bytes, s);
}
void scan_exclusive_diff_u32(const uint32_t *in, const uint32_t *sub, uint32_t *out, size_t n, void *tmp, size_t tmp_bytes,
			     hipStream_t s)
{
	if (n == 0)
		return;
	if (tmp_bytes < SC_MAX_BLOCKS * sizeof(uint32_t))
		throw HipError("scan: temporary storage too small");
	ScanJobs jobs{};
	jobs.j[0] = make_scan_job(in, out, n, static_cast<uint32_t *>(tmp), nullptr, sub);
	if (scan_lookback<0>(jobs, 1, tmp, tmp_bytes, s))
		return;
	KLAUNCH(k_scan_partials<0>, dim3(jobs.j[0].blocks, 1), dim3(SC_TPB), 0, s, jobs);
	KLAUNCH(k_scan_chunks<0>, dim3(jobs.j[0].blocks, 1), dim3(SC_TPB), 0, s, jobs);
}

template <int OP>
static void scan_exclusive_pair(const uint32_t *in0, uint32_t *out0, size_t n0, const uint32_t *in1, uint32_t *out1, size_t n1,
				void *tmp, size_t tmp_bytes, hipStream_t s)
{
	if (n0 == 0 || n1 == 0) {
		scan_exclusive<OP>(in0, out0, n0, tmp, tmp_bytes, s);
		scan_exclusive<OP>(in1, out1, n1, tmp, tmp_bytes, s);
		return;
	}
	if (tmp_bytes < 2 * SC_MAX_BLOCKS * sizeof(uint32_t))
		throw HipError("scan: temporary storage too small");
	ScanJobs jobs{};
	jobs.j[0] = make_scan_job(in0, out0, n0, static_cast<uint32_t *>(tmp));
	jobs.j[1] = make_scan_job(in1, out1, n1, static_cast<uint32_t *>(tmp) + SC_MAX_BLOCKS);
	if (scan_lookback<OP>(jobs, 2, tmp, tmp_bytes, s))
		return;
	const unsigned gx = std::max(jobs.j[0].blocks, jobs.j[1].blocks);
	KLAUNCH(k_scan_partials<OP>, dim3(gx, 2), dim3(SC_TPB), 0, s, jobs);
	KLAUNCH(k_scan_chunks<OP>, dim3(gx, 2), dim3(SC_TPB), 0, s, jobs);
}

void scan_exclusive_u32_pair(const uint32_t *in0, uint32_t *out0, size_t n0, const uint32_t *in1, uint32_t *out1, size_t n1,
			     void *tmp, size_t tmp_bytes, hipStream_t s)
{
	scan_exclusive_pair<0>(in0, out0, n0, in1, out1, n1, tmp, tmp_bytes, s);
}

void scan_exclusive_xor_u32_pair(const uint32_t *in0, uint32_t *out0, const uint32_t *in1, uint32_t *out1, size_t n, void *tmp,
				 size_t tmp_bytes, hipStream_t s)
{
	scan_exclusive_pair<2>(in0, out0, n, in1, out1, n, tmp, tmp_bytes, s);
}

void scan_exclusive_max_u32(const uint32_t *in, uint32_t *out, size_t n, void *tmp, size_t tmp_bytes, hipStream_t s)
{
	scan_exclusive<1>(in, out, n, tmp, tmp_bytes, s);
}

__global__ void __launch_bounds__(SC_TPB) k_totals_u32(uint64_t n, const uint32_t *__restrict__ a, const uint32_t *__restrict__ b,
						      unsigned long long *__restrict__ tot)
{
	__shared__ unsigned long long sa, sb;
	if (threadIdx.x == 0)
		sa = sb = 0;
	__syncthreads();
	unsigned long long x = 0, y = 0;
	for (uint64_t i = (uint64_t)blockIdx.x * SC_TPB + threadIdx.x; i < n; i += (uint64_t)gridDim.x * SC_TPB) {
		x += a[i];
		if (b)
			y += b[i];
	}
// ... 538 lines not shown
```

povu_amd/csrc/hip/tree_kernels.hip:

```cpp
#include "tree_kernels.hpp"

#include <cstdlib>

#include <algorithm>
#include <vector>

namespace povu_hip
{

#ifndef NIL
#define NIL POVU_NIL
#endif
static constexpr int TPB = 256;
static inline unsigned nblk(size_t n) { return (unsigned)((n + TPB - 1) / TPB); }
#define LAUNCH(k, n, s, ...)                                                                     \
	do {                                                                                     \
		if ((n) > 0) {                                                                   \
			hipLaunchKernelGGL(k, dim3(nblk(n)), dim3(TPB), 0, s, __VA_ARGS__);      \
			HIP_CHECK(hipGetLastError());                                            \
		}                                                                                \
	} while (0)

static unsigned rank_bucket_bits(size_t n)
{
	if (const char *ev = getenv("POVU_HIP_RANK_BITS"))
		return (unsigned)std::min(6, std::max(2, atoi(ev)));
	(void)n;
	return 3u;
}
static constexpr uint32_t PK_END = 0x1FFFFFFFu, PK_STOP = 0x80000000u;
static constexpr uint32_t P0_END = 0x3FFFFFFFu, P0_W = 0x40000000u, P0_HEAD = 0x80000000u;
static constexpr uint32_t FT_NONE = 0x7FFFFFFFu, FT_HASH = 0x80000000u;
__device__ __forceinline__ uint32_t bucket_splitter(uint32_t q, unsigned b) { return (q << b) | ((q * 0x9E3779B1u) >> (32u - b)); }
__device__ __forceinline__ bool is_splitter(uint32_t i, unsigned b) { return bucket_splitter(i >> b, b) == i; }
__device__ __forceinline__ uint32_t rank_pack(uint32_t nx, uint32_t w, unsigned b)
{
	(void)b;
	return (nx == NIL ? P0_END : nx) | ((w & 1u) ? P0_W : 0u);
}
__device__ __forceinline__ bool rank_l0_stop(uint32_t nx, unsigned b) { return nx == P0_END || is_splitter(nx, b); }

__device__ __forceinline__ uint32_t find_link_slot(const uint32_t *__restrict__ loff, const uint32_t *__restrict__ lle, uint32_t w,
						   uint32_t le)
{
	uint32_t lo = loff[w], hi = loff[w + 1];
	const uint32_t l0 = lo;
	if (hi - lo > 8) {
		while (lo < hi) {
			const uint32_t mid = (lo + hi) >> 1;
			if ((lle[mid] & LLE_ID) < le)
				lo = mid + 1;
			else
				hi = mid;
		}
		return lo - l0 + 1;
	}
	for (uint32_t j = lo; j < hi; j++)
		if ((lle[j] & LLE_ID) == le)
			return j - l0 + 1;
	return 0;
}
__device__ __forceinline__ void store2_unaligned(uint32_t *p, uint32_t a, uint32_t b)
{
	typedef uint32_t v2a __attribute__((ext_vector_type(2), aligned(4)));
	v2a v;
	v.x = a;
	v.y = b;
	*reinterpret_cast<v2a *>(p) = v;
}
__device__ __forceinline__ uint32_t arc_twin(const uint32_t *__restrict__ loff, const uint32_t *__restrict__ ladj,
					     const uint32_t *__restrict__ lle, uint32_t at)
{
	const uint32_t w = ladj[at];
	return loff[w] + find_link_slot(loff, lle, w, lle[at] & LLE_ID) - 1;
}
__device__ __forceinline__ ulonglong2 link_hash(uint32_t le)
{
	unsigned long long z = ((unsigned long long)le + 1ull) * 0x9E3779B97F4A7C15ull;
	z = (z ^ (z >> 30)) * 0xBF58476D1CE4E5B9ull;
	z = (z ^ (z >> 27)) * 0x94D049BB133111EBull;
	unsigned long long y = ((unsigned long long)le ^ 0x5851F42D4C957F2Dull) * 0xD6E8FEB86659FD93ull;
	y = (y ^ (y >> 33)) * 0xFF51AFD7ED558CCDull;
	y = (y ^ (y >> 33)) * 0xC4CEB9FE1A85EC53ull;
	return make_ulonglong2(z ^ (z >> 31), y ^ (y >> 33));
}
__device__ __forceinline__ ulonglong2 hx(const ulonglong2 a, const ulonglong2 b) { return make_ulonglong2(a.x ^ b.x, a.y ^ b.y); }
__device__ __forceinline__ bool hzero(const ulonglong2 a) { return (a.x | a.y) == 0ull; }
__device__ __forceinline__ bool heq(const ulonglong2 a, const ulonglong2 b) { return a.x == b.x && a.y == b.y; }
__global__ void k_tour_words(uint32_t nS, const uint32_t *__restrict__ loff, const uint32_t *__restrict__ ladj,
			     const uint32_t *__restrict__ lle, uint32_t *__restrict__ pk, unsigned b,
			     ulonglong2 *__restrict__ hside, uint32_t *__restrict__ ft)
{
	uint32_t S = BIDX * blockDim.x + threadIdx.x;
	if (S >= nS)
		return;
	const uint32_t lo = loff[S], hi = loff[S + 1];
	ulonglong2 h = make_ulonglong2(0ull, 0ull);
	uint32_t first = NIL;
	for (uint32_t at0 = lo; at0 < hi; at0 += 4) {
		const uint32_t rem = hi - at0;
		const uint4 lw4 = load4_unaligned(lle + at0), w4 = load4_unaligned(ladj + at0);
		const uint32_t lws[4] = {lw4.x, lw4.y, lw4.z, lw4.w}, ws[4] = {w4.x, w4.y, w4.z, w4.w};
		bool tree[4];
		uint2 o01[4];
		uint32_t se[4];
#pragma unroll
		for (uint32_t q = 0; q < 4; q++) {
			tree[q] = q < rem && (lws[q] & LLE_TREE);
			o01[q] = make_uint2(0u, 0u);
			se[q] = 0;
			if (tree[q]) {
				const uint32_t g2 = ws[q] & ~1u;
				o01[q] = *reinterpret_cast<const uint2 *>(loff + g2);
				se[q] = loff[g2 + 2];
			}
		}
		uint4 a[4];
#pragma unroll
		for (uint32_t q = 0; q < 4; q++) {
			a[q] = make_uint4(0u, 0u, 0u, 0u);
			if (tree[q] && se[q] - o01[q].x <= 8)
				a[q] = load4_unaligned(lle + o01[q].x);
// ... 1040 lines not shown
	const uint32_t o = d4.x == 2 * g + 1 ? 2 * g : 2 * g + 1, e = o ^ 1u;
	const uint32_t p = (e & 1u) ? d4.z : d4.x, slot_e = (e & 1u) ? d4.w : d4.y;
	auto child_behind = [&](uint32_t par, uint32_t lo, uint32_t n, uint32_t from) {
		for (uint32_t k = from; k <= n; k += 4) {
			const uint4 x = load4_unaligned(ladj + lo + k - 1);
			const uint32_t rem = n + 1 - k;
			const uint2 r0 = dps[x.x];
			const uint2 r1 = rem > 1 ? dps[x.y] : make_uint2(NIL, 0u);
			const uint2 r2 = rem > 2 ? dps[x.z] : make_uint2(NIL, 0u);
			const uint2 r3 = rem > 3 ? dps[x.w] : make_uint2(NIL, 0u);
			if (r0.x == par && r0.y == k)
				return x.x;
			if (r1.x == par && r1.y == k + 1)
				return x.y;
			if (r2.x == par && r2.y == k + 2)
				return x.z;
			if (r3.x == par && r3.y == k + 3)
				return x.w;
		}
		return NIL;
	};
	const uint2 s01 = *reinterpret_cast<const uint2 *>(loff + 2 * g);
	const uint32_t s2 = loff[2 * g + 2];
	const uint32_t lo_o = (o & 1u) ? s01.y : s01.x, n_o = ((o & 1u) ? s2 : s01.y) - lo_o;
	const uint32_t lo_e = (e & 1u) ? s01.y : s01.x, n_e = ((e & 1u) ? s2 : s01.y) - lo_e;
	const uint32_t c_o = child_behind(o, lo_o, n_o, 1u);
	const uint32_t ns_o = child_behind(e, lo_e, n_e, 1u);
	uint32_t after_e = NIL;
	if (p != NIL) {
		const uint32_t lo_p = loff[p], n_p = loff[p + 1] - lo_p;
		const uint32_t ns_e = child_behind(p, lo_p, n_p, slot_e + 1);
		after_e = ns_e != NIL ? 3 * (ns_e >> 1) : leave_event(p, dps[p].x == (p ^ 1u));
	}
	uint32_t enter = rank_pack(c_o != NIL ? 3 * (c_o >> 1) : A + 1, 0u, b);
	if (p == NIL) {
		const uint32_t comp = ckey[g];
		if (cproc[comp]) {
			enter |= P0_HEAD;
			heads[comp] = A;
		}
	}
	pk[A] = enter;
	if (ns_o != NIL) {
		pk[A + 1] = rank_pack(3 * (ns_o >> 1), 0u, b);
		pk[A + 2] = rank_pack(after_e, 0u, b);
		merged[g] = 0;
	} else {
		pk[A + 1] = rank_pack(after_e, 1u, b);
		pk[A + 2] = P0_END;
		merged[g] = 1;
	}
}

__global__ void k_tree_emit(uint32_t nS, const uint2 *__restrict__ erec, L0Ranks R, const uint8_t *__restrict__ merged,
			    const uint2 *__restrict__ dps, const uint32_t *__restrict__ ckey,
			    const uint32_t *__restrict__ cproc, const uint32_t *__restrict__ voff,
			    const unsigned long long *__restrict__ start_key, const uint32_t *__restrict__ gid_s,
			    uint32_t *__restrict__ t_gid, uint8_t *__restrict__ t_flags, uint32_t *__restrict__ t_par,
			    uint32_t *__restrict__ t_size, uint32_t *__restrict__ t_depth, uint32_t *__restrict__ side_tidx,
			    uint32_t C, uint32_t *__restrict__ c_ntree, uint32_t *__restrict__ ordcnt, uint32_t *__restrict__ hi0,
			    uint32_t *__restrict__ mpre, uint32_t *__restrict__ srccnt, uint32_t *__restrict__ sdl,
			    uint32_t *__restrict__ incnt)
{
	uint32_t S = BIDX * blockDim.x + threadIdx.x;
	if (S == 0) {
		const uint32_t T = 2 * (nS >> 1) + C;
		hi0[T] = NIL;
		srccnt[T] = srccnt[T + 1] = 0;
		incnt[T] = incnt[T + 1] = 0;
	}
	if (S < C) {
		const uint32_t Nr = 2 * (voff[S + 1] - voff[S]), tr = 2 * voff[S] + S;
		if (!cproc[S]) {
			c_ntree[S] = 0;
			t_size[tr + Nr] = 0;
			srccnt[tr + Nr] = 0;
			incnt[tr + Nr] = 0;
		} else {
			const uint32_t hr = start_key[S] != ~0ull ? 1u : 0u;
			c_ntree[S] = Nr + hr;
			if (hr) {
				t_gid[tr] = NIL;
				t_flags[tr] = 2;
				t_par[tr] = NIL;
				t_size[tr] = Nr + 1;
				incnt[tr] = 0;
				if (t_depth)
					t_depth[tr] = 0;
				mpre[tr] = tr;
				ordcnt[tr] = 0;
				hi0[tr] = NIL;
			} else {
				t_size[tr + Nr] = 0;
				srccnt[tr + Nr] = 0;
				incnt[tr + Nr] = 0;
			}
		}
	}
	const uint32_t g = S;
	if (g >= (nS >> 1))
		return;
	const uint32_t c = ckey[g], v0 = voff[c];
	const uint32_t tb = 2 * v0 + c;
	if (!cproc[c]) {
		const uint32_t t = tb + 2 * (g - v0);
		store2_unaligned(t_size + t, 0u, 0u);
		store2_unaligned(srccnt + t, 0u, 0u);
		store2_unaligned(incnt + t, 0u, 0u);
		*reinterpret_cast<uint2 *>(side_tidx + 2 * g) = make_uint2(NIL, NIL);
		return;
	}
	const uint32_t Nh = 2 * (voff[c + 1] - v0), hd = start_key[c] != ~0ull ? 1u : 0u;
	const bool fin = *R.fin != 0;
	const uint4 r01 = load4_unaligned(reinterpret_cast<const uint32_t *>(erec + 3 * g));
	const uint2 ent = rank_l0_pair(R, make_uint2(r01.x, r01.y), fin);
	const uint2 lv_o = make_uint2(rank_l0_a(R, make_uint2(r01.z, r01.w), fin), 0u);
	const uint4 d4 = *reinterpret_cast<const uint4 *>(dps + 2 * g);
	const uint32_t o = d4.x == 2 * g + 1 ? 2 * g : 2 * g + 1, e = o ^ 1u;
	const uint32_t p = (e & 1u) ? d4.z : d4.x;
	const uint32_t pre_e = Nh - ent.x, depth_e = 0u - ent.y;
	uint32_t lv_e = lv_o.x;
	if (!merged[g]) {
		lv_e = rank_l0_a(R, erec[3 * g + 2], fin);
	}
	const uint32_t size_o = ent.x - 1 - lv_o.x, size_e = ent.x - lv_e;
	uint32_t par_e;
	if (p == NIL)
		par_e = hd ? 0u : NIL;
	else {
		par_e = hd + (Nh - rank_l0_a(R, erec[3 * (p >> 1)], fin)) + (dps[p].x == (p ^ 1u) ? 1u : 0u);
	}
	const uint32_t l = hd + pre_e, t = tb + l;
	const uint32_t gid = gid_s[g];
	store2_unaligned(t_gid + t, gid, gid);
	t_flags[t] = (uint8_t)(e & 1u);
	t_flags[t + 1] = (uint8_t)((o & 1u) | TF_BLACK);
	store2_unaligned(t_par + t, par_e, l);
	store2_unaligned(t_size + t, size_e, size_o);
	store2_unaligned(incnt + t, 0u, 0u);
	if (t_depth)
		store2_unaligned(t_depth + t, depth_e + hd, depth_e + 1 + hd);
	store2_unaligned(mpre + t, tb + (depth_e + hd) + (Nh + hd) - l - size_e, tb + (depth_e + 1 + hd) + (Nh + hd) - (l + 1) - size_o);
	*reinterpret_cast<uint2 *>(side_tidx + 2 * g) = (e & 1u) ? make_uint2(t + 1, t) : make_uint2(t, t + 1);
	if (sdl) {
		const uint32_t gray = (size_e - 1 - size_o) / 2, black = (size_o + 1) / 2, gs = v0 + pre_e / 2;
		if (gray) {
			atomicAdd(&sdl[gs], gray);
			atomicAdd(&sdl[gs + black], 0u - gray - black);
			atomicAdd(&sdl[gs + size_e / 2], black);
		}
	}
}
#ifndef POVU_BE_ITER
#define POVU_BE_ITER 8
#endif
static constexpr uint32_t BE_ITER = POVU_BE_ITER, BE_SIDES = TPB * BE_ITER;
template <bool EMIT>
__device__ __forceinline__ uint32_t side_back_edges(uint32_t S, uint32_t p, uint32_t at,
						    const uint32_t *__restrict__ loff, const uint32_t *__restrict__ ladj,
						    const uint2 *__restrict__ dps, const uint32_t *__restrict__ side_tidx,
// ... 11 lines not shown
			b_src[at + n] = p;
			b_tgt[at + n] = tgt;
			b_ord[at + n] = n;
			atomicAdd(&incnt[tgt], 1u);
		} else {
			highest = min(highest, tgt);
			if (n < 2)
				first2[n] = tgt;
		}
		n++;
	};
	if (lo == hi) {
		if (p == root || t_par[p] != 0)
			out(root);
		return n;
	}
	const uint32_t dp = dps[S].x;
	bool loop_seen = false;
	for (uint32_t k0 = lo; k0 < hi; k0 += 4) {
		const uint4 o4 = load4_unaligned(ladj + k0);
		const uint32_t rem = hi - k0;
		const uint32_t os[4] = {o4.x, o4.y, o4.z, o4.w};
		const uint32_t xs[4] = {side_tidx[o4.x], rem > 1 ? side_tidx[o4.y] : NIL, rem > 2 ? side_tidx[o4.z] : NIL,
					rem > 3 ? side_tidx[o4.w] : NIL};
#pragma unroll
		for (uint32_t q = 0; q < 4; q++) {
			if (q >= rem)
				break;
			const uint32_t k = k0 + q, o = os[q], x = xs[q];
			if (o == (S ^ 1)) {
				if (dp == o && !loop_seen)
					out(x);
				loop_seen = true;
				continue;
			}
			if (x > p || o == dp)
				continue;
			bool dup = false;
			if (dupflag) {
				dup = dupflag[k] != 0;
			} else {
				for (uint32_t j = lo; j < k; j++)
					if (ladj[j] == o) {
						dup = true;
						break;
					}
			}
			if (!dup)
				out(x);
		}
	}
	return n;
}
__global__ void __launch_bounds__(TPB) k_back_edges(uint32_t nS, const uint32_t *__restrict__ loff, const uint32_t *__restrict__ ladj,
						     const uint2 *__restrict__ dps, const uint32_t *__restrict__ side_tidx,
						     const uint32_t *__restrict__ ckey, const uint32_t *__restrict__ voff,
						     const uint32_t *__restrict__ t_par, uint32_t *__restrict__ total_out,
						     uint32_t *__restrict__ b_src, uint32_t *__restrict__ b_tgt,
						     uint32_t *__restrict__ b_ord, const uint8_t *__restrict__ dupflag,
						     uint32_t *__restrict__ ordcnt, uint32_t *__restrict__ hi0, uint32_t *__restrict__ incnt,
						     uint32_t cap)
{
	const uint32_t S0 = BIDX * BE_SIDES + threadIdx.x;
	__shared__ uint32_t first2[BE_ITER][TPB][2];
	__shared__ uint8_t cnt8[BE_ITER][TPB];
	uint32_t n = 0;
	for (uint32_t it = 0; it < BE_ITER; it++) {
		const uint32_t S = S0 + it * TPB;
		const uint32_t p = S < nS ? side_tidx[S] : NIL;
		uint32_t k = 0;
		if (p != NIL) {
			uint32_t highest = NIL;
			k = side_back_edges<false>(S, p, 0, loff, ladj, dps, side_tidx, ckey, voff, t_par, b_src, b_tgt, b_ord, dupflag, incnt, highest,
						   first2[it][threadIdx.x]);
			ordcnt[p] = k;
			hi0[p] = highest;
			n += k;
		}
		cnt8[it][threadIdx.x] = (uint8_t)min(k, 255u);
	}
	__shared__ uint32_t wsum[TPB / 64], base;
	const uint32_t lane = threadIdx.x & 63u, wave = threadIdx.x >> 6;
	uint32_t inc = n;
	for (int off = 1; off < 64; off <<= 1) {
		const uint32_t y = __shfl_up(inc, off);
		if ((int)lane >= off)
			inc += y;
	}
	if (lane == 63)
		wsum[wave] = inc;
	__syncthreads();
	uint32_t before = 0, all = 0;
	for (uint32_t w = 0; w < TPB / 64; w++) {
		if (w < wave)
			before += wsum[w];
		all += wsum[w];
	}
	if (threadIdx.x == 0)
		base = all ? atomicAdd(total_out, all) : 0u;
	__syncthreads();
	if (!n || base + all > cap)
		return;
	uint32_t at = base + before + inc - n;
	for (uint32_t it = 0; it < BE_ITER; it++) {
		const uint32_t k = cnt8[it][threadIdx.x];
		if (!k)
			continue;
		const uint32_t S = S0 + it * TPB, p = side_tidx[S];
		if (k <= 2) {
			for (uint32_t j = 0; j < k; j++) {
				const uint32_t tgt = first2[it][threadIdx.x][j];
				b_src[at + j] = p;
				b_tgt[at + j] = tgt;
				b_ord[at + j] = j;
				atomicAdd(&incnt[tgt], 1u);
			}
			at += k;
		} else {
			uint32_t unused = NIL;
			at += side_back_edges<true>(S, p, at, loff, ladj, dps, side_tidx, ckey, voff, t_par, b_src, b_tgt, b_ord, dupflag, incnt, unused,
						    nullptr);
		}
	}
}

__global__ void k_edge_id_weights(uint32_t nS, const uint32_t *__restrict__ loff, const uint32_t *__restrict__ ladj,
				  const uint2 *__restrict__ dps,
				  const uint32_t *__restrict__ side_tidx, const uint32_t *__restrict__ ckey,
// ... 257 lines not shown
			publish_words(w, WordSrc{{n_over}}, 1, s);
			const HostScratch::Token published = tw.host->mark(s);
			enqueue_events();
			tw.host->wait(published);
			n_big = *w;
			events_done = n_big == 0;
		} else {
			n_big = tw.host->read_u32(n_over, s);
		}
		big_list = over_list;
	}
	if (n_big) {
		if (!tw.walk_inline) {
			if (!tw.walk_arena)
				throw HipError("class walk: no arena for the wave walk's arrays (internal)");
			const WalkBytes wb(2 * (size_t)V + 2);
			tw.walk_arena->reserve(walk_workspace_bytes(V));
			tw.wrec = reinterpret_cast<decltype(tw.wrec)>(tw.walk_arena->take<char>(wb.rec));
			tw.wstk = reinterpret_cast<decltype(tw.wstk)>(tw.walk_arena->take<char>(wb.stk));
			tw.wpar = reinterpret_cast<decltype(tw.wpar)>(tw.walk_arena->take<char>(wb.par));
		}
		uint32_t *pool_top = pw.err + 7, *walk_err = pw.err + 8;
		LAUNCH(k_class_recs, nS, s, nS, cs.loff, cs.ladj, cstate, cs.ckey, tw.cproc, tw.wadj, tw.wrec, tw.wpar);
		const uint32_t route = getenv("POVU_HIP_WALK_ROUTE") ? (uint32_t)atoi(getenv("POVU_HIP_WALK_ROUTE")) : 0u;
		const uint32_t pool_cap = (uint32_t)std::min<size_t>(3 * (size_t)nS, 0xFFFFFFF0u);
		hipStream_t s2 = tw.walk_stream ? tw.walk_stream : s;
		if (s2 != s) {
			HIP_CHECK(hipEventRecord(tw.walk_fork, s));
			HIP_CHECK(hipStreamWaitEvent(s2, tw.walk_fork, 0));
		}
		KLAUNCH(k_class_walk_wave<false>, dim3(n_big), dim3(64), 0, s2, n_big, big_list, tw.wrec, tw.wadj, tw.wpar, tw.wstk, pool_top, pool_cap,
			walk_err, nS, route);
		KLAUNCH(k_class_walk_wave<true>, dim3(n_big), dim3(64), 0, s, n_big, big_list, tw.wrec, tw.wadj, tw.wpar, tw.wstk, pool_top, pool_cap,
			walk_err, nS, route);
		if (s2 != s) {
			HIP_CHECK(hipEventRecord(tw.walk_join, s2));
			HIP_CHECK(hipStreamWaitEvent(s, tw.walk_join, 0));
		}
		LAUNCH(k_walk_finish, nS, s, nS, tw.wpar, cstate, cs.loff, cs.ladj, tw.dps);
		if (tw.host->read_u32(walk_err, s))
			throw HipError("class walk: stack pool exhausted (internal sizing bug)");
	}
	tm.end(5);

	tm.begin("tree_preorder");
	(void)max_side_links;
	if (!events_done)
		enqueue_events();
	const L0Ranks evr = list_rank_splitters<true, true>(n_events, bitsE, tw.evt, pw.err + 13, C, rb, s);
	(void)event_lists;
	tm.end(40);

	tm.begin("tree_emit");
	LAUNCH(k_tree_emit, std::max(V, C), s, nS, tw.evt, evr, merged, tw.dps, cs.ckey, tw.cproc, cs.voff, start_key, cs.gid_s, sw.t_gid, sw.t_flags,
	       sw.t_par, sw.t_size, (sw.hairpins || sw.want_depth) ? sw.t_depth : nullptr, tw.side_tidx, C, sw.c_ntree, pw.lsz, pw.hi0, pw.mpre, pw.dlt,
	       pw.sdl, pw.incnt);
	pw.sdl_filled = true;
	const uint8_t *dupflag = nullptr;
	if (max_side_links > 64 && E) {
		const uint32_t n_slots = 2 * E;
		uint32_t *k1 = (uint32_t *)tw.xval, *k2 = k1 + n_slots, *v1 = (uint32_t *)tw.xps, *v2 = v1 + n_slots;
		uint32_t *side_of = (uint32_t *)tw.evt;
		LAUNCH(k_slot_keys, n_slots, s, n_slots, cs.ladj, k1, v1);
		sort_pairs_u32(k1, k2, v1, v2, n_slots, bits_for(nS), pw.sort_tmp, pw.sort_tmp_bytes, s);
		LAUNCH(k_slot_side, nS, s, nS, cs.loff, side_of);
		LAUNCH(k_gather_keys, n_slots, s, n_slots, v2, side_of, k1);
		sort_pairs_u32(k1, k2, v2, v1, n_slots, bits_for(nS), pw.sort_tmp, pw.sort_tmp_bytes, s);
		LAUNCH(k_dup_flags, n_slots, s, n_slots, k2, v1, cs.ladj, tw.dvis_slots);
		dupflag = tw.dvis_slots;
	}
	tw.last_dupflag = dupflag;
	uint32_t *nb0_dev = pw.err + 6;
	KLAUNCH(k_back_edges, dim3((nS + BE_SIDES - 1) / BE_SIDES), dim3(TPB), 0, s, nS, cs.loff, cs.ladj, tw.dps, tw.side_tidx, cs.ckey,
		cs.voff, sw.t_par, nb0_dev, pw.b_src, pw.b_tgt, pw.b_ord, dupflag, pw.lsz, pw.hi0, pw.incnt,
		(uint32_t)std::min<size_t>(pw.nb_cap, 0xFFFFFFFFu));
	tm.end(6);
	return NB0_ON_DEVICE;
}

}
```

povu_amd/hip.py:

```python
from __future__ import annotations

import ctypes as C
import os
from dataclasses import dataclass
from typing import Dict, List, Optional

import numpy as np

_HERE = os.path.dirname(os.path.abspath(__file__))


class HipUnavailable(RuntimeError):
    pass


class GuardBandError(RuntimeError):
    """A device-wide primitive wrote outside its output (raised by its unit-test hook, which guards every output)."""


SCAN_SUM, SCAN_MAX, SCAN_U64, SCAN_U8, SCAN_DIFF, SCAN_XOR_PAIR, SCAN_XOR_U128 = range(7)
SCAN_IN_PLACE, SCAN_N_DEV = 0x100, 0x200
SEG_MIN, SEG_FIRST_LESS, SEG_LAST_LESS = range(3)


def lib_path() -> str:
    return os.path.join(_HERE, "lib", "libpovu_hip.so")


class _Opts(C.Structure):
    _fields_ = [("rank", C.c_uint32), ("world", C.c_uint32), ("flags", C.c_uint32)]


class _SubTree(C.Structure):
    _fields_ = [("n_total", C.c_uint32), ("n_flubble_like", C.c_uint32), ("n_concealed", C.c_uint32), ("n_midi", C.c_uint32),
                ("n_smothered", C.c_uint32), ("fam", C.POINTER(C.c_uint8)), ("or1", C.POINTER(C.c_uint8)),
                ("or2", C.POINTER(C.c_uint8)), ("route", C.POINTER(C.c_uint8)), ("id1", C.POINTER(C.c_uint32)),
                ("id2", C.POINTER(C.c_uint32)), ("child_off", C.POINTER(C.c_uint32)), ("child", C.POINTER(C.c_uint32))]


class _Tree(C.Structure):
    _fields_ = [("component_id", C.c_uint32), ("n_vtx", C.c_uint32), ("n_links", C.c_uint32),
                ("n_pvst", C.c_uint32), ("a_id", C.POINTER(C.c_uint32)), ("z_id", C.POINTER(C.c_uint32)),
                ("a_or", C.POINTER(C.c_uint8)), ("z_or", C.POINTER(C.c_uint8)), ("parent", C.POINTER(C.c_uint32)),
                ("n_hairpins", C.c_uint32), ("hairpins", C.POINTER(C.c_uint64))]


class _ShardInfo(C.Structure):
    _fields_ = [("n_vtx", C.c_uint32), ("n_links", C.c_uint32), ("n_components", C.c_uint32), ("weight", C.c_uint64),
                ("bytes", C.c_size_t), ("device_ptr", C.c_void_p)]


class _MultiRank(C.Structure):
    _fields_ = [("device", C.c_int), ("n_vtx", C.c_uint32), ("n_links", C.c_uint32), ("n_components", C.c_uint32),
                ("shard_bytes", C.c_uint64), ("recv_ms", C.c_double), ("csr_ms", C.c_double), ("decompose_ms", C.c_double),
                ("sink_ms", C.c_double), ("h2d", C.c_uint64), ("d2h", C.c_uint64), ("peer_out", C.c_uint64),
                ("peer_in", C.c_uint64)]


class _WalkOpts(C.Structure):
    _fields_ = [("max_walks", C.c_uint32), ("max_steps", C.c_uint32), ("max_expansions", C.c_uint32), ("flags", C.c_uint32)]


class _Walks(C.Structure):
    _fields_ = [("n_queries", C.c_uint64), ("n_walks", C.c_uint64), ("n_steps", C.c_uint64),
                ("walk_off", C.POINTER(C.c_uint32)), ("step_off", C.POINTER(C.c_uint32)), ("step_id", C.POINTER(C.c_uint32)),
                ("step_or", C.POINTER(C.c_uint8)), ("status", C.POINTER(C.c_uint8)), ("n_tier2", C.c_uint64),
                ("device_ms", C.c_double)]


class _TravOpts(C.Structure):
    _fields_ = [("max_steps", C.c_uint32), ("flags", C.c_uint32)]


# ... 142 lines not shown
    l.povu_hip_forest_raw.argtypes = [C.c_void_p, C.POINTER(C.c_void_p), C.POINTER(C.c_size_t), C.POINTER(C.c_uint64),
                                      C.POINTER(C.c_uint64)]
    l.povu_hip_forest_walks.restype = C.POINTER(_Walks)
    l.povu_hip_forest_walks.argtypes = [C.c_void_p, C.c_void_p, C.POINTER(_WalkOpts), C.c_char_p, C.c_size_t]
    l.povu_hip_walks_free.argtypes = [C.POINTER(_Walks)]
    l.povu_hip_paths_upload.restype = C.c_int
    l.povu_hip_paths_upload.argtypes = [C.c_void_p, C.c_uint32, C.c_void_p, C.c_void_p, C.c_void_p, C.c_char_p, C.c_size_t]
    l.povu_hip_forest_traversals.restype = C.POINTER(_Traversals)
    l.povu_hip_forest_traversals.argtypes = [C.c_void_p, C.c_void_p, C.POINTER(_TravOpts), C.c_char_p, C.c_size_t]
    l.povu_hip_traversals_free.argtypes = [C.POINTER(_Traversals)]
    l.povu_hip_forest_first.restype = C.c_uint64
    l.povu_hip_segments_upload.argtypes = [C.c_void_p, C.c_uint32, C.c_void_p, C.c_void_p, C.c_char_p, C.c_size_t]
    l.povu_hip_segments_upload.restype = C.c_int
    l.povu_hip_call.argtypes = [C.c_void_p, C.POINTER(_Sites), C.POINTER(_CallRefs), C.POINTER(C.c_uint32), C.POINTER(_TravOpts),
                                C.c_char_p, C.c_size_t]
    l.povu_hip_call.restype = C.POINTER(_CallsNested)
    l.povu_hip_call_profile.argtypes = [C.c_void_p, C.POINTER(_Sites), C.POINTER(_CallRefs), C.POINTER(C.c_uint32), C.POINTER(_TravOpts),
                                        C.POINTER(_ProfileOpts), C.c_char_p, C.c_size_t]
    l.povu_hip_call_profile.restype = C.POINTER(_CallsNested)
    l.povu_hip_calls_vcf_profile.argtypes = [C.POINTER(_CallsNested), C.POINTER(_Sites), C.POINTER(_CallNames), C.POINTER(C.c_char_p),
                                             C.c_char_p, C.c_char_p, C.c_uint32, C.c_uint32, C.POINTER(C.c_size_t)]
    l.povu_hip_calls_vcf_profile.restype = C.c_void_p
    l.povu_hip_calls_vcf_rest.argtypes = [C.POINTER(_CallsNested), C.POINTER(_Sites), C.POINTER(_CallNames), C.POINTER(C.c_char_p),
                                          C.c_char_p, C.POINTER(C.c_char_p), C.c_uint32, C.c_uint32, C.c_uint32, C.POINTER(C.c_size_t)]
    l.povu_hip_calls_vcf_rest.restype = C.c_void_p
    l.povu_hip_calls_free.argtypes = [C.POINTER(_Calls)]
    l.povu_hip_call_names_make.argtypes = [C.c_uint32, C.POINTER(C.c_char_p), C.c_uint32, C.POINTER(C.c_char_p), C.c_char_p,
                                           C.c_size_t]
    l.povu_hip_call_names_make.restype = C.POINTER(_CallNames)
    l.povu_hip_call_names_free.argtypes = [C.POINTER(_CallNames)]
    l.povu_hip_sites_of_docs.argtypes = [C.c_void_p, C.c_uint32]
    l.povu_hip_sites_of_docs.restype = C.POINTER(_Sites)
    l.povu_hip_forest_sites.argtypes = [C.c_void_p]
    l.povu_hip_forest_sites.restype = C.POINTER(_Sites)
    l.povu_hip_sites_free.argtypes = [C.POINTER(_Sites)]
    l.povu_hip_calls_vcf.argtypes = [C.POINTER(_Calls), C.POINTER(_Sites), C.POINTER(_CallNames), C.POINTER(C.c_char_p), C.c_char_p,
                                     C.c_char_p, C.c_uint32, C.POINTER(C.c_size_t)]
    l.povu_hip_calls_vcf.restype = C.c_void_p
    l.povu_hip_forest_first.argtypes = [C.c_void_p, C.c_uint32]
    l.povu_hip_forest_pvst_text.restype = C.c_void_p
    l.povu_hip_forest_pvst_text.argtypes = [C.c_void_p, C.c_uint32, C.POINTER(C.c_size_t)]
    l.povu_hip_buffer_free.argtypes = [C.c_void_p]
    l.povu_hip_last_stage_times.restype = C.c_int
    l.povu_hip_last_stage_times.argtypes = [C.c_void_p, C.POINTER(_StageTime), C.c_int]
    l.povu_hip_last_seq_redo.restype = C.c_uint32
    l.povu_hip_last_seq_redo.argtypes = [C.c_void_p]
    l.povu_hip_last_links_processed.restype = C.c_uint64
    l.povu_hip_last_links_processed.argtypes = [C.c_void_p]
    l.povu_hip_debug_components.restype = C.c_int
    l.povu_hip_debug_components.argtypes = [C.c_void_p, C.c_void_p, C.c_void_p]
    l.povu_hip_debug_tree.restype = C.c_int
    l.povu_hip_debug_tree.argtypes = [C.c_void_p, C.c_uint32, C.POINTER(C.c_uint32), C.c_void_p, C.c_void_p,
                                      C.c_void_p, C.c_void_p]
    l.povu_hip_last_black_only_classes.restype = C.c_int
    l.povu_hip_last_black_only_classes.argtypes = [C.c_void_p]
    l.povu_hip_last_crossings.restype = C.c_int
    l.povu_hip_last_crossings.argtypes = [C.c_void_p, C.POINTER(C.c_uint32)]
    l.povu_hip_last_laminar_check_ran.restype = C.c_int
    l.povu_hip_last_laminar_check_ran.argtypes = [C.c_void_p]
    l.povu_hip_debug_edge_ids.restype = C.c_int
    l.povu_hip_debug_edge_ids.argtypes = [C.c_void_p, C.c_uint32, C.POINTER(C.c_uint32), C.c_void_p]
    l.povu_hip_debug_stack.restype = C.c_int
    l.povu_hip_debug_stack.argtypes = [C.c_void_p, C.c_uint32, C.POINTER(C.c_uint32), C.c_void_p, C.c_void_p,
                                       C.c_void_p]
    l.povu_hip_version.restype = C.c_char_p
    l.povu_hip_debug_scan.restype = C.c_int
    l.povu_hip_debug_scan.argtypes = [C.c_void_p, C.c_int, C.c_void_p, C.c_void_p, C.c_size_t, C.c_void_p, C.c_void_p,
                                      C.c_size_t]
    l.povu_hip_debug_sort.restype = C.c_int
    l.povu_hip_debug_sort.argtypes = [C.c_void_p, C.c_void_p, C.c_void_p, C.c_size_t, C.c_uint, C.c_void_p, C.c_void_p]
    l.povu_hip_debug_compact.restype = C.c_int
    l.povu_hip_debug_compact.argtypes = [C.c_void_p, C.c_void_p, C.c_size_t, C.c_void_p, C.POINTER(C.c_uint32)]
    l.povu_hip_debug_totals.restype = C.c_int
    l.povu_hip_debug_totals.argtypes = [C.c_void_p, C.c_void_p, C.c_void_p, C.c_size_t, C.POINTER(C.c_uint64)]
    l.povu_hip_debug_segtree.restype = C.c_int
    l.povu_hip_debug_segtree.argtypes = [C.c_void_p, C.c_void_p, C.c_size_t, C.c_void_p, C.c_size_t, C.c_void_p, C.c_void_p,
                                         C.POINTER(C.c_uint32)]
    l.povu_hip_debug_bitrank.restype = C.c_int
    l.povu_hip_debug_bitrank.argtypes = [C.c_void_p, C.c_void_p, C.c_size_t, C.c_void_p, C.c_size_t, C.c_void_p, C.c_void_p,
                                         C.c_void_p]
    l.povu_hip_debug_append.restype = C.c_int
    l.povu_hip_debug_append.argtypes = [C.c_void_p, C.c_void_p, C.c_size_t, C.c_void_p, C.POINTER(C.c_uint32)]
    l.povu_hip_debug_list_rank.restype = C.c_int
    l.povu_hip_debug_list_rank.argtypes = [C.c_void_p, C.c_uint32, C.c_void_p, C.c_void_p, C.c_void_p, C.c_uint32,
                                           C.c_int, C.c_uint32, C.c_void_p, C.c_void_p]
    l.povu_hip_workspace_estimate.restype = C.c_uint64
    l.povu_hip_workspace_estimate.argtypes = [C.c_uint32, C.c_uint32, C.c_uint32]
    l.povu_hip_prewarm.restype = C.c_int
    l.povu_hip_prewarm.argtypes = [C.c_void_p, C.c_uint32, C.c_uint32, C.c_char_p, C.c_size_t]
    l.povu_hip_leaf_workspace_estimate.restype = C.c_uint64
    l.povu_hip_leaf_workspace_estimate.argtypes = [C.c_uint32, C.c_uint32]
    l.povu_hip_lpt_assign.restype = C.c_int
    l.povu_hip_lpt_assign.argtypes = [C.c_void_p, C.c_uint32, C.c_uint32, C.c_void_p]
    l.povu_hip_shard_partition.restype = C.c_void_p
    l.povu_hip_shard_partition.argtypes = [C.c_void_p, C.c_uint32, C.c_char_p, C.c_size_t]
    l.povu_hip_shards_world.restype = C.c_uint32
    l.povu_hip_shards_world.argtypes = [C.c_void_p]
    l.povu_hip_shards_total_components.restype = C.c_uint32
    l.povu_hip_shards_total_components.argtypes = [C.c_void_p]
    l.povu_hip_shards_get.restype = C.c_int
    l.povu_hip_shards_get.argtypes = [C.c_void_p, C.c_uint32, C.POINTER(_ShardInfo)]
    l.povu_hip_shards_times.restype = C.c_int
    l.povu_hip_shards_times.argtypes = [C.c_void_p, C.POINTER(C.c_double)]
    l.povu_hip_shards_export.restype = C.c_int
    l.povu_hip_shards_export.argtypes = [C.c_void_p, C.c_void_p, C.c_uint32, C.c_void_p]
    l.povu_hip_shards_free.argtypes = [C.c_void_p]
# ... 704 lines not shown
    def seq_redo_count(self) -> int:
        return int(self._lib.povu_hip_last_seq_redo(self._ctx))

    def links_processed(self) -> int:
        return int(self._lib.povu_hip_last_links_processed(self._ctx))

    @staticmethod
    def _prim_rc(rc: int, primitive: str):
        if rc == 5:
            raise GuardBandError(f"{primitive}: a guard band around a device output changed")
        if rc:
            raise RuntimeError(f"{primitive}: debug hook failed ({rc})")

    def debug_scan(self, a, op: int = 0, b=None, in_place: bool = False):
        a = np.ascontiguousarray(a, dtype=np.uint64 if op == 2 else np.uint32)
        out = np.empty_like(a)
        name = ("scan_exclusive_u32", "scan_exclusive_max_u32", "scan_exclusive_u64")[op]
        if b is None:
            rc = self._lib.povu_hip_debug_scan(self._ctx, op | (SCAN_IN_PLACE if in_place else 0), a.ctypes.data,
                                               out.ctypes.data, a.size, None, None, 0)
            self._prim_rc(rc, name + (" (in place)" if in_place else ""))
            return out
        b = np.ascontiguousarray(b, dtype=np.uint32)
        out2 = np.empty_like(b)
        rc = self._lib.povu_hip_debug_scan(self._ctx, op, a.ctypes.data, out.ctypes.data, a.size, b.ctypes.data,
                                           out2.ctypes.data, b.size)
        self._prim_rc(rc, "scan_exclusive_u32_pair" if op == 0 else name)
        return out, out2

    def debug_scan_u8(self, a, b=None):
        a = np.ascontiguousarray(a, dtype=np.uint8)
        out = np.empty(a.size, dtype=np.uint32)
        if b is None:
            rc = self._lib.povu_hip_debug_scan(self._ctx, SCAN_U8, a.ctypes.data, out.ctypes.data, a.size, None, None, 0)
            self._prim_rc(rc, "scan_exclusive_u8")
            return out
        b = np.ascontiguousarray(b, dtype=np.uint8)
        out2 = np.empty(b.size, dtype=np.uint32)
        rc = self._lib.povu_hip_debug_scan(self._ctx, SCAN_U8, a.ctypes.data, out.ctypes.data, a.size, b.ctypes.data,
                                           out2.ctypes.data, b.size)
        self._prim_rc(rc, "scan_exclusive_u8 (two jobs)")
        return out, out2

    def debug_scan_diff(self, a, sub):
        a = np.ascontiguousarray(a, dtype=np.uint32)
        sub = np.ascontiguousarray(sub, dtype=np.uint32)
        assert a.size == sub.size
        out = np.empty_like(a)
        rc = self._lib.povu_hip_debug_scan(self._ctx, SCAN_DIFF, a.ctypes.data, out.ctypes.data, a.size, sub.ctypes.data,
                                           None, sub.size)
        self._prim_rc(rc, "scan_exclusive_diff_u32")
        return out

    def debug_scan_xor_pair(self, a, b):
        a = np.ascontiguousarray(a, dtype=np.uint32)
        b = np.ascontiguousarray(b, dtype=np.uint32)
        assert a.size == b.size
        out, out2 = np.empty_like(a), np.empty_like(b)
        rc = self._lib.povu_hip_debug_scan(self._ctx, SCAN_XOR_PAIR, a.ctypes.data, out.ctypes.data, a.size,
                                           b.ctypes.data, out2.ctypes.data, b.size)
        self._prim_rc(rc, "scan_exclusive_xor_u32_pair")
        return out, out2

    def debug_scan_xor_u128(self, a, n_dev=None):
        a = np.ascontiguousarray(a, dtype=np.uint64)
        assert a.ndim == 2 and a.shape[1] == 2
        out = np.empty_like(a)
        op = SCAN_XOR_U128 | (SCAN_N_DEV if n_dev is not None else 0)
        rc = self._lib.povu_hip_debug_scan(self._ctx, op, a.ctypes.data, out.ctypes.data, a.shape[0], None, None,
                                           n_dev or 0)
        self._prim_rc(rc, "scan_exclusive_xor_u128")
        return out if n_dev is None else out[:min(n_dev + 1, a.shape[0])]

    def debug_sort(self, keys, vals, bits: int):
        keys = np.ascontiguousarray(keys, dtype=np.uint32)
        vals = np.ascontiguousarray(vals, dtype=np.uint32)
        assert keys.size == vals.size
        ko, vo = np.empty_like(keys), np.empty_like(vals)
        rc = self._lib.povu_hip_debug_sort(self._ctx, keys.ctypes.data, vals.ctypes.data, keys.size, bits,
                                           ko.ctypes.data, vo.ctypes.data)
        self._prim_rc(rc, "sort_pairs_u32")
        return ko, vo

    def debug_compact(self, flags):
        flags = np.ascontiguousarray(flags, dtype=np.uint8)
        out = np.empty(flags.size, dtype=np.uint32)
        cnt = C.c_uint32(0)
        rc = self._lib.povu_hip_debug_compact(self._ctx, flags.ctypes.data, flags.size, out.ctypes.data, C.byref(cnt))
        self._prim_rc(rc, "compact_flagged_u8")
        if cnt.value > flags.size:
            raise RuntimeError(f"compact_flagged_u8: count {cnt.value} of {flags.size} flags")
        return out[:cnt.value], int(cnt.value)

    def debug_totals(self, a, b=None):
        a = np.ascontiguousarray(a, dtype=np.uint32)
        tot = (C.c_uint64 * 2)()
        if b is not None:
            b = np.ascontiguousarray(b, dtype=np.uint32)
            assert a.size == b.size
        rc = self._lib.povu_hip_debug_totals(self._ctx, a.ctypes.data, b.ctypes.data if b is not None else None, a.size, tot)
        self._prim_rc(rc, "totals_u32")
        return int(tot[0]) if b is None else (int(tot[0]), int(tot[1]))

    def debug_segtree(self, values, queries, want_tree: bool = False):
        values = np.ascontiguousarray(values, dtype=np.uint32)
        queries = np.ascontiguousarray(queries, dtype=np.uint32).reshape(-1, 4)
# ... 12 lines not shown

    def debug_bitrank(self, flags, positions):
        flags = np.ascontiguousarray(flags, dtype=np.uint8)
        positions = np.ascontiguousarray(positions, dtype=np.uint32)
        rank, test = np.empty(positions.size, dtype=np.uint32), np.empty(positions.size, dtype=np.uint32)
        records = np.empty((flags.size // 64 + 2, 4), dtype=np.uint32)
        rc = self._lib.povu_hip_debug_bitrank(self._ctx, flags.ctypes.data, flags.size, positions.ctypes.data, positions.size,
                                              rank.ctypes.data, test.ctypes.data, records.ctypes.data)
        self._prim_rc(rc, "bit-rank directory (bitrank_store_wave / bitrank_build)")
        return rank, test, records

    def debug_append(self, flags):
        flags = np.ascontiguousarray(flags, dtype=np.uint8)
        out = np.empty(flags.size, dtype=np.uint32)
        cnt = C.c_uint32(0)
        rc = self._lib.povu_hip_debug_append(self._ctx, flags.ctypes.data, flags.size, out.ctypes.data, C.byref(cnt))
        self._prim_rc(rc, "append_in_order")
        if cnt.value > flags.size:
            raise RuntimeError(f"append_in_order: length {cnt.value} of {flags.size} flags")
        return out[:cnt.value], int(cnt.value)

    def debug_list_rank(self, nxt, w, heads, events: bool = False, bits: int = 0):
        nxt = np.ascontiguousarray(nxt, dtype=np.uint32)
        w = np.ascontiguousarray(w, dtype=np.uint8)
        heads = np.ascontiguousarray(heads, dtype=np.uint32)
        ra = np.zeros(nxt.size, dtype=np.uint32)
        rb = np.zeros(nxt.size, dtype=np.uint32)
        rc = self._lib.povu_hip_debug_list_rank(self._ctx, nxt.size, nxt.ctypes.data, w.ctypes.data,
                                                heads.ctypes.data if heads.size else None, heads.size,
                                                1 if events else 0, bits, ra.ctypes.data, rb.ctypes.data)
        if rc:
            raise RuntimeError(f"debug_list_rank failed ({rc})")
        return (ra, rb) if events else ra

    def debug_components(self, n_vtx: int):
        comp = np.zeros(n_vtx, dtype=np.uint32)
        loc = np.zeros(n_vtx, dtype=np.uint32)
        if self._lib.povu_hip_debug_components(self._ctx, comp.ctypes.data, loc.ctypes.data) != 0:
            raise RuntimeError("no decompose state")
        return comp, loc

    def debug_tree(self, comp: int):
        n = C.c_uint32(0)
        if self._lib.povu_hip_debug_tree(self._ctx, comp, C.byref(n), None, None, None, None) != 0:
            raise RuntimeError("no decompose state")
        gid = np.zeros(n.value, dtype=np.uint32)
        typ = np.zeros(n.value, dtype=np.uint8)
        par = np.zeros(n.value, dtype=np.uint32)
        cls = np.zeros(n.value, dtype=np.uint32)
        self._lib.povu_hip_debug_tree(self._ctx, comp, C.byref(n), gid.ctypes.data, typ.ctypes.data, par.ctypes.data,
                                      cls.ctypes.data)
        return dict(gid=gid, typ=typ & 3, black=(typ >> 2) & 1, par=par, cls=cls)

    def last_black_only_classes(self) -> bool:
        return bool(self._lib.povu_hip_last_black_only_classes(self._ctx))

    def last_crossings(self):
        o = (C.c_uint32 * 2)()
        if self._lib.povu_hip_last_crossings(self._ctx, o) != 0:
            raise RuntimeError("povu_hip_last_crossings failed")
        return int(o[0]), int(o[1])

    def last_laminar_check_ran(self) -> bool:
        return bool(self._lib.povu_hip_last_laminar_check_ran(self._ctx))

    def debug_edge_ids(self, comp: int):
        n = C.c_uint32(0)
        rc = self._lib.povu_hip_debug_edge_ids(self._ctx, comp, C.byref(n), None)
        if rc != 0:
            raise RuntimeError("no parallel-tree state" if rc == 3 else "no decompose state")
        ids = np.zeros(n.value, dtype=np.uint32)
        if self._lib.povu_hip_debug_edge_ids(self._ctx, comp, C.byref(n), ids.ctypes.data) != 0:
            raise RuntimeError("povu_hip_debug_edge_ids failed")
        return ids

    def debug_stack(self, comp: int):
        n = C.c_uint32(0)
        if self._lib.povu_hip_debug_stack(self._ctx, comp, C.byref(n), None, None, None) != 0:
            raise RuntimeError("no decompose state")
        vtx = np.zeros(n.value, dtype=np.uint32)
        cls = np.zeros(n.value, dtype=np.uint32)
        ns = np.zeros(n.value, dtype=np.uint32)
        self._lib.povu_hip_debug_stack(self._ctx, comp, C.byref(n), vtx.ctypes.data, cls.ctypes.data, ns.ctypes.data)
        return dict(tree_vtx=vtx, cls=cls, next_seen=ns)


class MultiDecomposer:

    def __init__(self, devices):
        self._lib = load_lib()
        if self._lib.povu_hip_device_count() <= 0:
            raise HipUnavailable("no HIP device visible: the decompose path has no CPU fallback")
        devs = (C.c_int * len(devices))(*[int(d) for d in devices])
        err = C.create_string_buffer(512)
        self._h = self._lib.povu_hip_multi_create(devs, len(devices), err, 512)
        if not self._h:
            raise HipUnavailable(err.value.decode())
        self.world = len(devices)

    def close(self):
        if getattr(self, "_h", None):
            self._lib.povu_hip_multi_destroy(self._h)
            self._h = None

    def __del__(self):
        self.close()
# ... 43 lines not shown
```

Measured before the change: 3.160 billion.

## Store per-vertex order and source counts as bytes when degree bound fits

When the maximum per-vertex count bound fits in a byte, ordcnt and srccnt are stored as uint8 arrays instead of uint32. The tree-emit, back-edge and bracket-extra kernels are templated on the element type, and new scan variants read u8 input with a u32 subtrahend or pair a u32 scan with a u8 scan. The aim is to cut memory traffic for these per-tree-vertex arrays across several kernels and scans. It adds template instantiations and an environment override, and relies on the bound check being correct to avoid truncation.

```diff
diff --git a/include/povu_hip.h b/include/povu_hip.h
--- a/include/povu_hip.h
+++ b/include/povu_hip.h
@@ -396,6 +396,7 @@
 int povu_hip_last_stage_times(const povu_hip_ctx *ctx, povu_hip_stage_time *out, int max);
 uint32_t povu_hip_last_seq_redo(const povu_hip_ctx *ctx);
 int povu_hip_last_black_only_classes(const povu_hip_ctx *ctx);
+int povu_hip_last_narrow_counts(const povu_hip_ctx *ctx);
 int povu_hip_last_laminar_check_ran(const povu_hip_ctx *ctx);
 int povu_hip_last_crossings(povu_hip_ctx *ctx, uint32_t out[2]);
 uint64_t povu_hip_last_links_processed(const povu_hip_ctx *ctx);
@@ -414,6 +415,8 @@
 #define POVU_HIP_SCAN_DIFF 4
 #define POVU_HIP_SCAN_XOR_PAIR 5
 #define POVU_HIP_SCAN_XOR_U128 6
+#define POVU_HIP_SCAN_DIFF_U8 7
+#define POVU_HIP_SCAN_MIXED_PAIR 8
 #define POVU_HIP_SCAN_IN_PLACE 0x100
 #define POVU_HIP_SCAN_N_DEV 0x200
 int povu_hip_debug_scan(povu_hip_ctx *ctx, int op, const uint32_t *in, uint32_t *out, size_t n, const uint32_t *in2,
diff --git a/povu_amd/csrc/hip/common.hpp b/povu_amd/csrc/hip/common.hpp
--- a/povu_amd/csrc/hip/common.hpp
+++ b/povu_amd/csrc/hip/common.hpp
@@ -296,6 +296,10 @@
 		       size_t tmp_bytes, hipStream_t s);
 void scan_exclusive_diff_u32(const uint32_t *in, const uint32_t *sub, uint32_t *out, size_t n, void *tmp, size_t tmp_bytes,
 			     hipStream_t s);
+void scan_exclusive_diff_u8_u32(const uint8_t *in8, const uint32_t *sub, uint32_t *out, size_t n, void *tmp, size_t tmp_bytes,
+				hipStream_t s);
+void scan_exclusive_u32_u8_pair(const uint32_t *in0, uint32_t *out0, size_t n0, const uint8_t *in1, uint32_t *out1, size_t n1,
+				void *tmp, size_t tmp_bytes, hipStream_t s);
 void scan_exclusive_xor_u128(const ulonglong2 *in, ulonglong2 *out, size_t n, void *tmp, size_t tmp_bytes, hipStream_t s,
 			     const uint32_t *n_dev = nullptr);
 size_t scan_tmp_bytes(size_t n);
diff --git a/povu_amd/csrc/hip/context.hpp b/povu_amd/csrc/hip/context.hpp
--- a/povu_amd/csrc/hip/context.hpp
+++ b/povu_amd/csrc/hip/context.hpp
@@ -220,6 +220,7 @@
 	PassPlan plan;
 	uint32_t C = 0, seq_redo = 0;
 	bool mixed = false, redo_pvst_only = false, stack_export_pending = false;
+	bool narrow_counts = false;
 };
 
 struct povu_hip_ctx {
diff --git a/povu_amd/csrc/hip/debug_hooks.hip b/povu_amd/csrc/hip/debug_hooks.hip
--- a/povu_amd/csrc/hip/debug_hooks.hip
+++ b/povu_amd/csrc/hip/debug_hooks.hip
@@ -88,31 +88,32 @@
 {
 	const int kind = op & 0xFF;
 	const bool in_place = (op & POVU_HIP_SCAN_IN_PLACE) != 0, with_len = (op & POVU_HIP_SCAN_N_DEV) != 0;
-	if (!ctx || kind > POVU_HIP_SCAN_XOR_U128 || (op & ~(0xFF | POVU_HIP_SCAN_IN_PLACE | POVU_HIP_SCAN_N_DEV)))
+	if (!ctx || kind > POVU_HIP_SCAN_MIXED_PAIR || (op & ~(0xFF | POVU_HIP_SCAN_IN_PLACE | POVU_HIP_SCAN_N_DEV)))
 		return 1;
 	if (kind == POVU_HIP_SCAN_U8) {
 		if ((n && (!in || !out)) || (in2 && n2 && !out2))
 			return 1;
-	} else if (!in || !out || (in2 && !out2 && kind != POVU_HIP_SCAN_DIFF)) {
+	} else if (!in || !out || (in2 && !out2 && kind != POVU_HIP_SCAN_DIFF && kind != POVU_HIP_SCAN_DIFF_U8)) {
 		return 1;
 	}
 	if ((in_place && (kind > POVU_HIP_SCAN_U64 || in2)) || (with_len && kind != POVU_HIP_SCAN_XOR_U128) ||
-	    ((kind == POVU_HIP_SCAN_DIFF || kind == POVU_HIP_SCAN_XOR_PAIR) && !in2))
-		return 1;
-	try {
-		HIP_CHECK(hipSetDevice(ctx->device));
-		hipStream_t s = ctx->stream;
-		const size_t e_in = kind == POVU_HIP_SCAN_U8 ? 1 : kind == POVU_HIP_SCAN_U64 ? 8 : kind == POVU_HIP_SCAN_XOR_U128 ? 16 : 4;
+	    ((kind == POVU_HIP_SCAN_DIFF || kind == POVU_HIP_SCAN_XOR_PAIR || kind == POVU_HIP_SCAN_DIFF_U8 || kind == POVU_HIP_SCAN_MIXED_PAIR) && !in2))
+		return 1;
+	try {
+		HIP_CHECK(hipSetDevice(ctx->device));
+		hipStream_t s = ctx->stream;
+		const size_t e_in = (kind == POVU_HIP_SCAN_U8 || kind == POVU_HIP_SCAN_DIFF_U8) ? 1 : kind == POVU_HIP_SCAN_U64 ? 8 : kind == POVU_HIP_SCAN_XOR_U128 ? 16 : 4;
+		const size_t e_in2 = kind == POVU_HIP_SCAN_DIFF_U8 ? 4 : kind == POVU_HIP_SCAN_MIXED_PAIR ? 1 : e_in;
 		const size_t e_out = kind == POVU_HIP_SCAN_U64 ? 8 : kind == POVU_HIP_SCAN_XOR_U128 ? 16 : 4;
-		const bool pair = in2 && (kind == POVU_HIP_SCAN_SUM || kind == POVU_HIP_SCAN_U8 || kind == POVU_HIP_SCAN_XOR_PAIR);
-		const bool second_in = pair || kind == POVU_HIP_SCAN_DIFF;
-		const size_t m = !second_in ? 0 : (kind == POVU_HIP_SCAN_SUM || kind == POVU_HIP_SCAN_U8) ? n2 : n;
+		const bool pair = in2 && (kind == POVU_HIP_SCAN_SUM || kind == POVU_HIP_SCAN_U8 || kind == POVU_HIP_SCAN_XOR_PAIR || kind == POVU_HIP_SCAN_MIXED_PAIR);
+		const bool second_in = pair || kind == POVU_HIP_SCAN_DIFF || kind == POVU_HIP_SCAN_DIFF_U8;
+		const size_t m = !second_in ? 0 : (kind == POVU_HIP_SCAN_SUM || kind == POVU_HIP_SCAN_U8 || kind == POVU_HIP_SCAN_MIXED_PAIR) ? n2 : n;
 		const size_t tb = kind == POVU_HIP_SCAN_U64 ? scan_exclusive_u64_tmp(n) * 8 : scan_tmp_bytes(std::max(n, m));
 		const uint32_t len = (uint32_t)n2;
 		Arena ar;
 		DbgOut o1{n * e_out}, o2{m * e_out, DBG_GUARD_BYTE, pair};
 		DbgScratch scr{tb};
-		DbgIn<char> i1{reinterpret_cast<const char *>(in), n * e_in, !in_place}, i2{reinterpret_cast<const char *>(in2), m * e_in, second_in};
+		DbgIn<char> i1{reinterpret_cast<const char *>(in), n * e_in, !in_place}, i2{reinterpret_cast<const char *>(in2), m * e_in2, second_in};
 		DbgIn<uint32_t> ilen{&len, 1, with_len};
 		dbg_carve(ar, s, o1, o2, scr, i1, i2, ilen);
 		if (in_place)
@@ -138,6 +139,12 @@
 					  pair ? reinterpret_cast<const uint8_t *>(di2) : nullptr, pair ? o2.data<uint32_t>() : nullptr, m, tmp, tb, s);
 			break;
 		case POVU_HIP_SCAN_DIFF: scan_exclusive_diff_u32(w1, w2, o1.data<uint32_t>(), n, tmp, tb, s); break;
+		case POVU_HIP_SCAN_DIFF_U8:
+			scan_exclusive_diff_u8_u32(reinterpret_cast<const uint8_t *>(di), w2, o1.data<uint32_t>(), n, tmp, tb, s);
+			break;
+		case POVU_HIP_SCAN_MIXED_PAIR:
+			scan_exclusive_u32_u8_pair(w1, o1.data<uint32_t>(), n, reinterpret_cast<const uint8_t *>(di2), o2.data<uint32_t>(), m, tmp, tb, s);
+			break;
 		case POVU_HIP_SCAN_XOR_PAIR: scan_exclusive_xor_u32_pair(w1, o1.data<uint32_t>(), w2, o2.data<uint32_t>(), n, tmp, tb, s); break;
 		default:
 			scan_exclusive_xor_u128(reinterpret_cast<const ulonglong2 *>(di), o1.data<ulonglong2>(), n, tmp, tb, s, ilen.dev);
diff --git a/povu_amd/csrc/hip/par_kernels.hip b/povu_amd/csrc/hip/par_kernels.hip
--- a/povu_amd/csrc/hip/par_kernels.hip
+++ b/povu_amd/csrc/hip/par_kernels.hip
@@ -3,6 +3,7 @@
 
 #include <algorithm>
 #include <cstdlib>
+#include <type_traits>
 
 namespace povu_hip
 {
@@ -43,9 +44,11 @@
 	uint32_t t = BIDX * blockDim.x + threadIdx.x;
 	if (t >= T)
 		return;
-	srccnt[t] = 0;
-	if (t == T - 1)
-		srccnt[T] = srccnt[T + 1] = 0;
+	if (srccnt) {
+		srccnt[t] = 0;
+		if (t == T - 1)
+			srccnt[T] = srccnt[T + 1] = 0;
+	}
 	if (cov) {
 		hi0[t] = NIL;
 		cov[t] = 0;
@@ -286,14 +289,15 @@
 		tsimp[tile] = tile < ntiles ? ns : 0u;
 	}
 }
+template <typename OC, typename SC>
 __global__ void __launch_bounds__(TPB) k_bracket_extra(uint32_t T, uint32_t NB0_host, const uint32_t *__restrict__ nb0_dev, uint32_t ntiles,
 							uint32_t nb_cap, const uint8_t *__restrict__ capf,
 							const uint32_t *__restrict__ tcap, const uint8_t *__restrict__ simp,
 							const uint32_t *__restrict__ tsimp, const uint32_t *__restrict__ cap_tgt,
 							const RootOf root_of, uint32_t *__restrict__ b_src, uint32_t *__restrict__ b_tgt,
-							const uint32_t *__restrict__ ordcnt, const uint32_t *__restrict__ gsize,
+							const OC *__restrict__ ordcnt, const uint32_t *__restrict__ gsize,
 							const uint32_t *__restrict__ mpre, uint32_t *__restrict__ incnt,
-							uint32_t *__restrict__ srccnt)
+							SC *__restrict__ srccnt)
 {
 	const uint32_t NB0 = nb0_dev ? *nb0_dev : NB0_host, ncap = tcap[ntiles];
 	if ((uint64_t)NB0 + ncap + tsimp[ntiles] > nb_cap)
@@ -325,7 +329,12 @@
 	uint4 oc = make_uint4(0u, 0u, 0u, 0u), gs = oc, mp = oc;
 	if (ordcnt) {
 		if (v0 + 4 <= T) {
-			oc = *reinterpret_cast<const uint4 *>(ordcnt + v0);
+			if constexpr (sizeof(OC) == 1) {
+				const uint32_t w = *reinterpret_cast<const uint32_t *>(ordcnt + v0);
+				oc = make_uint4(w & 0xFFu, (w >> 8) & 0xFFu, (w >> 16) & 0xFFu, w >> 24);
+			} else {
+				oc = *reinterpret_cast<const uint4 *>(ordcnt + v0);
+			}
 			gs = *reinterpret_cast<const uint4 *>(gsize + v0);
 			mp = *reinterpret_cast<const uint4 *>(mpre + v0);
 		} else {
@@ -358,7 +367,7 @@
 				atomicAdd(&incnt[root], 1u);
 		}
 		if (ordcnt && gsv[j])
-			srccnt[mpv[j]] = ocv[j] + (c ? 1u : 0u) + (sm ? 1u : 0u);
+			srccnt[mpv[j]] = (SC)(ocv[j] + (c ? 1u : 0u) + (sm ? 1u : 0u));
 	}
 }
 __global__ void k_bracket_order(uint32_t NB, uint32_t NB0, uint32_t ncap, uint32_t nsimp, const uint32_t *__restrict__ b_src,
@@ -1021,6 +1030,10 @@
 	pw.nb_cap = NB;
 	auto skip = [](auto **p) { *p = nullptr; };
 	take1(T + 2, pw.hi0, pw.mpre, pw.dlt, pw.incnt, pw.lsz);
+	if (groups & 1) {
+		pw.ordcnt8 = reinterpret_cast<uint8_t *>(pw.lsz);
+		pw.srccnt8 = reinterpret_cast<uint8_t *>(pw.dlt);
+	}
 	take1(NB + 2, pw.b_src, pw.b_tgt, pw.b_ord);
 	take1(V + 4, pw.sdl);
 	take1(16, pw.err);
@@ -1134,13 +1147,14 @@
 
 	tm.begin("par_setup");
 	const bool lean = dense_nb0 >= 0 && !want_hp;
+	const bool narrow_oc = dense_nb0 >= 0 && pw.narrow_ordcnt, narrow_sc = narrow_oc && pw.narrow_srccnt;
 	if (lean) {
 		pw.gsize = sw.t_size;
 		pw.gpar = sw.t_par;
 	} else {
 		LAUNCH(k_tcomp_vertices, V, s, V, T, cs.ckey, cs.voff, pw.t_comp);
 		LAUNCH(k_globalize, T, s, T, pw.t_comp, cs.voff, sw.c_ntree, sw.t_par, sw.t_size, pw.gpar, pw.gsize, pw.t_root, pw.hi0,
-		       dense_nb0 >= 0 ? nullptr : pw.cov, sw.t_depth, pw.mpre, pw.incnt, pw.dlt);
+		       dense_nb0 >= 0 ? nullptr : pw.cov, sw.t_depth, pw.mpre, pw.incnt, narrow_sc ? nullptr : pw.dlt);
 	}
 	const RootOf root_of{lean ? nullptr : pw.t_root, cs.voff, C};
 	uint32_t NB0;
@@ -1162,7 +1176,9 @@
 	uint4 *brec = reinterpret_cast<uint4 *>(pw.psA);
 	uint32_t *brec_cnt = reinterpret_cast<uint32_t *>(pw.f8a);
 	uint32_t *pscov = pw.psB;
-	if (dense_nb0 >= 0)
+	if (narrow_oc)
+		scan_exclusive_diff_u8_u32(pw.ordcnt8, pw.incnt, pscov, (size_t)T + 1, pw.scan_tmp, pw.scan_tmp_bytes, s);
+	else if (dense_nb0 >= 0)
 		scan_exclusive_diff_u32(pw.lsz, pw.incnt, pscov, (size_t)T + 1, pw.scan_tmp, pw.scan_tmp_bytes, s);
 	else
 		scan(pw.cov, pscov, (size_t)T + 1);
@@ -1181,10 +1197,22 @@
 	uint32_t *extra = pw.host->take<uint32_t>(4);
 	publish_words(extra, WordSrc{{tcap + ntiles, tsimp + ntiles, pw.err + 5, pw.err + 6}}, 4, s);
 	const HostScratch::Token extra_ready = pw.host->mark(s);
-	LAUNCH(k_bracket_extra, ((size_t)T + 3) / 4, s, T, NB0, dense_nb0 == NB0_ON_DEVICE ? pw.err + 6 : nullptr, ntiles,
-	       (uint32_t)std::min<size_t>(pw.nb_cap, 0xFFFFFFFFu), capf, tcap, simp, tsimp, pw.cap_tgt, root_of, pw.b_src, pw.b_tgt,
-	       dense_nb0 >= 0 ? pw.lsz : nullptr, pw.gsize, pw.mpre, pw.incnt, srccnt);
-	if (dense_nb0 >= 0)
+	auto bracket_extra = [&](auto *ordcnt, auto *sc) {
+		using OC = std::remove_const_t<std::remove_pointer_t<decltype(ordcnt)>>;
+		using SC = std::remove_pointer_t<decltype(sc)>;
+		LAUNCH((k_bracket_extra<OC, SC>), ((size_t)T + 3) / 4, s, T, NB0, dense_nb0 == NB0_ON_DEVICE ? pw.err + 6 : nullptr, ntiles,
+		       (uint32_t)std::min<size_t>(pw.nb_cap, 0xFFFFFFFFu), capf, tcap, simp, tsimp, pw.cap_tgt, root_of, pw.b_src, pw.b_tgt,
+		       ordcnt, pw.gsize, pw.mpre, pw.incnt, sc);
+	};
+	if (narrow_sc)
+		bracket_extra((const uint8_t *)pw.ordcnt8, pw.srccnt8);
+	else if (narrow_oc)
+		bracket_extra((const uint8_t *)pw.ordcnt8, srccnt);
+	else
+		bracket_extra(dense_nb0 >= 0 ? (const uint32_t *)pw.lsz : nullptr, srccnt);
+	if (narrow_sc)
+		scan_exclusive_u32_u8_pair(pw.incnt, pw.psin, (size_t)T + 1, pw.srccnt8, bstart, (size_t)T + 1, pw.scan_tmp, pw.scan_tmp_bytes, s);
+	else if (dense_nb0 >= 0)
 		scan2(pw.incnt, pw.psin, (size_t)T + 1, srccnt, bstart, (size_t)T + 1);
 	pw.host->wait(extra_ready);
 	if (dense_nb0 == NB0_ON_DEVICE) {
diff --git a/povu_amd/csrc/hip/par_kernels.hpp b/povu_amd/csrc/hip/par_kernels.hpp
--- a/povu_amd/csrc/hip/par_kernels.hpp
+++ b/povu_amd/csrc/hip/par_kernels.hpp
@@ -36,6 +36,8 @@
 	uint32_t *hi0, *cov, *psA, *psB, *flagC, *psC;
 	uint8_t *f8a, *f8b, *f8c, *f8d;
 	uint32_t *cap_tgt, *mpre, *dlt, *dlt_ps, *incnt, *psin, *topi, *lsz, *gcls;
+	uint8_t *ordcnt8, *srccnt8;
+	bool narrow_ordcnt = false, narrow_srccnt = false;
 	uint32_t *sdl;
 	bool sdl_filled = false;
 	uint32_t *vals_t, *vals_t2;
diff --git a/povu_amd/csrc/hip/povu_hip.hip b/povu_amd/csrc/hip/povu_hip.hip
--- a/povu_amd/csrc/hip/povu_hip.hip
+++ b/povu_amd/csrc/hip/povu_hip.hip
@@ -814,6 +814,7 @@
 	pw.cproc_ps = sw.tables + 2 * ((size_t)C + 1);
 	ctx->tw.cproc = sw.tables + 3 * ((size_t)C + 1);
 	pw.soff = sw.tables + 4 * ((size_t)C + 1);
+	pw.narrow_ordcnt = pw.narrow_srccnt = false;
 	if (p.seq_tree) {
 		lanes.init(s);
 		tm.begin("tree_seq");
@@ -821,6 +822,11 @@
 		launch_seq_components(sw, s);
 		tm.end(1);
 	} else {
+		const char *ev = getenv("POVU_HIP_WIDE_COUNTS");
+		const int wide = ev ? atoi(ev) : 0;
+		const bool fits = std::max<uint32_t>(gstats[0], 1u) + 2u <= 255u;
+		pw.narrow_ordcnt = fits && wide != 1;
+		pw.narrow_srccnt = pw.narrow_ordcnt && wide != 2;
 		dense_nb0 = run_parallel_tree(ctx->cs, sw, pw, ctx->tw, C, t.event_lists, gstats[0], p.big_class_dfs, p.sparse_splitters, tm, s);
 	}
 	pw.all_vertex_classes = p.all_vertex_classes;
@@ -1195,6 +1201,7 @@
 			ctx->ws_sub.release();
 		stage_times(ctx, tm, *f);
 		ctx->last = LastPass{true, p, C, out.nbad, out.mixed, out.redo_pvst_only, out.stack_export_pending};
+		ctx->last.narrow_counts = !p.all_seq && !p.seq_tree && ctx->pw.narrow_ordcnt;
 		if (p.world == 1 && ctx->shard_comp_ids.empty()) {
 			f->walk_ctx = ctx;
 			f->walk_gen = g.gen;
@@ -1531,6 +1538,11 @@
 
 extern "C" uint64_t povu_hip_last_links_processed(const povu_hip_ctx *ctx) { return ctx ? ctx->last_links : 0; }
 
+extern "C" int povu_hip_last_narrow_counts(const povu_hip_ctx *ctx)
+{
+	return ctx && ctx->last.valid && ctx->last.narrow_counts ? 1 : 0;
+}
+
 extern "C" int povu_hip_last_black_only_classes(const povu_hip_ctx *ctx)
 {
 	return ctx && ctx->last.valid && !ctx->last.plan.all_seq && ctx->pw.black_only_used ? 1 : 0;
diff --git a/povu_amd/csrc/hip/primitives.hip b/povu_amd/csrc/hip/primitives.hip
--- a/povu_amd/csrc/hip/primitives.hip
+++ b/povu_amd/csrc/hip/primitives.hip
@@ -56,12 +56,20 @@
 		auto bytes4 = [](uint32_t w) {
 			return sc_op<MAX>(sc_op<MAX>(w & 0xFFu, (w >> 8) & 0xFFu), sc_op<MAX>((w >> 16) & 0xFFu, w >> 24));
 		};
+		const uint32_t *__restrict__ sub = J.sub;
 		for (size_t i = b0 + 16 * (size_t)threadIdx.x; i < w1; i += 16 * SC_TPB) {
 			const uint4 a = *reinterpret_cast<const uint4 *>(in8 + i);
 			fold4(make_uint4(bytes4(a.x), bytes4(a.y), bytes4(a.z), bytes4(a.w)));
+			if (sub) {
+#pragma unroll
+				for (int q = 0; q < 4; q++) {
+					const uint4 c = *reinterpret_cast<const uint4 *>(sub + i + 4 * q);
+					acc -= c.x + c.y + c.z + c.w;
+				}
+			}
 		}
 		for (size_t i = w1 + threadIdx.x; i < b1; i += SC_TPB)
-			acc = sc_op<MAX>(acc, in8[i]);
+			acc = sc_op<MAX>(acc, in8[i] - (sub ? sub[i] : 0u));
 	} else {
 		const uint32_t *__restrict__ sub = J.sub;
 		const size_t w1 = b0 + ((b1 - b0) & ~size_t(3));
@@ -89,9 +97,13 @@
 			const uint2 a = *reinterpret_cast<const uint2 *>(in8 + e0);
 			v[0] = a.x & 0xFFu, v[1] = (a.x >> 8) & 0xFFu, v[2] = (a.x >> 16) & 0xFFu, v[3] = a.x >> 24;
 			v[4] = a.y & 0xFFu, v[5] = (a.y >> 8) & 0xFFu, v[6] = (a.y >> 16) & 0xFFu, v[7] = a.y >> 24;
+			if (J.sub) {
+				const uint4 c = *reinterpret_cast<const uint4 *>(J.sub + e0), d = *reinterpret_cast<const uint4 *>(J.sub + e0 + 4);
+				v[0] -= c.x, v[1] -= c.y, v[2] -= c.z, v[3] -= c.w, v[4] -= d.x, v[5] -= d.y, v[6] -= d.z, v[7] -= d.w;
+			}
 		} else {
 			for (int k = 0; k < SC_ITEMS; k++)
-				v[k] = e0 + k < b1 ? in8[e0 + k] : 0u;
+				v[k] = e0 + k < b1 ? in8[e0 + k] - (J.sub ? J.sub[e0 + k] : 0u) : 0u;
 		}
 	} else if (e0 + SC_ITEMS <= b1) {
 		const uint32_t *__restrict__ in = J.in;
@@ -223,6 +235,15 @@
 			v[q][0] = a[q].x & 0xFFu, v[q][1] = (a[q].x >> 8) & 0xFFu, v[q][2] = (a[q].x >> 16) & 0xFFu, v[q][3] = a[q].x >> 24;
 			v[q][4] = a[q].y & 0xFFu, v[q][5] = (a[q].y >> 8) & 0xFFu, v[q][6] = (a[q].y >> 16) & 0xFFu, v[q][7] = a[q].y >> 24;
 		}
+		if (J.sub) {
+			const uint32_t *__restrict__ sub = J.sub + b0 + (size_t)threadIdx.x * SC_ITEMS;
+#pragma unroll
+			for (int q = 0; q < LB_SUB; q++) {
+				const uint4 c = *reinterpret_cast<const uint4 *>(sub + q * SC_TILE), d = *reinterpret_cast<const uint4 *>(sub + q * SC_TILE + 4);
+				v[q][0] -= c.x, v[q][1] -= c.y, v[q][2] -= c.z, v[q][3] -= c.w;
+				v[q][4] -= d.x, v[q][5] -= d.y, v[q][6] -= d.z, v[q][7] -= d.w;
+			}
+		}
 	} else {
 #pragma unroll
 		for (int q = 0; q < LB_SUB; q++)
@@ -435,6 +456,41 @@
 		return;
 	KLAUNCH(k_scan_partials<0>, dim3(jobs.j[0].blocks, 1), dim3(SC_TPB), 0, s, jobs);
 	KLAUNCH(k_scan_chunks<0>, dim3(jobs.j[0].blocks, 1), dim3(SC_TPB), 0, s, jobs);
+}
+
+void scan_exclusive_diff_u8_u32(const uint8_t *in8, const uint32_t *sub, uint32_t *out, size_t n, void *tmp, size_t tmp_bytes,
+				hipStream_t s)
+{
+	if (n == 0)
+		return;
+	if (tmp_bytes < SC_MAX_BLOCKS * sizeof(uint32_t))
+		throw HipError("scan: temporary storage too small");
+	ScanJobs jobs{};
+	jobs.j[0] = make_scan_job(nullptr, out, n, static_cast<uint32_t *>(tmp), in8, sub);
+	if (scan_lookback<0>(jobs, 1, tmp, tmp_bytes, s))
+		return;
+	KLAUNCH(k_scan_partials<0>, dim3(jobs.j[0].blocks, 1), dim3(SC_TPB), 0, s, jobs);
+	KLAUNCH(k_scan_chunks<0>, dim3(jobs.j[0].blocks, 1), dim3(SC_TPB), 0, s, jobs);
+}
+
+void scan_exclusive_u32_u8_pair(const uint32_t *in0, uint32_t *out0, size_t n0, const uint8_t *in1, uint32_t *out1, size_t n1,
+				void *tmp, size_t tmp_bytes, hipStream_t s)
+{
+	if (n0 == 0 || n1 == 0) {
+		scan_exclusive<0>(in0, out0, n0, tmp, tmp_bytes, s);
+		scan_exclusive_u8(in1, out1, n1, nullptr, nullptr, 0, tmp, tmp_bytes, s);
+		return;
+	}
+	if (tmp_bytes < 2 * SC_MAX_BLOCKS * sizeof(uint32_t))
+		throw HipError("scan: temporary storage too small");
+	ScanJobs jobs{};
+	jobs.j[0] = make_scan_job(in0, out0, n0, static_cast<uint32_t *>(tmp));
+	jobs.j[1] = make_scan_job(nullptr, out1, n1, static_cast<uint32_t *>(tmp) + SC_MAX_BLOCKS, in1);
+	if (scan_lookback<0>(jobs, 2, tmp, tmp_bytes, s))
+		return;
+	const unsigned gx = std::max(jobs.j[0].blocks, jobs.j[1].blocks);
+	KLAUNCH(k_scan_partials<0>, dim3(gx, 2), dim3(SC_TPB), 0, s, jobs);
+	KLAUNCH(k_scan_chunks<0>, dim3(gx, 2), dim3(SC_TPB), 0, s, jobs);
 }
 
 template <int OP>
diff --git a/povu_amd/csrc/hip/tree_kernels.hip b/povu_amd/csrc/hip/tree_kernels.hip
--- a/povu_amd/csrc/hip/tree_kernels.hip
+++ b/povu_amd/csrc/hip/tree_kernels.hip
@@ -3,6 +3,7 @@
 #include <cstdlib>
 
 #include <algorithm>
+#include <type_traits>
 #include <vector>
 
 namespace povu_hip
@@ -68,6 +69,8 @@
 	v.y = b;
 	*reinterpret_cast<v2a *>(p) = v;
 }
+__device__ __forceinline__ void zero2(uint32_t *p) { store2_unaligned(p, 0u, 0u); }
+__device__ __forceinline__ void zero2(uint8_t *p) { p[0] = p[1] = 0; }
 __device__ __forceinline__ uint32_t arc_twin(const uint32_t *__restrict__ loff, const uint32_t *__restrict__ ladj,
 					     const uint32_t *__restrict__ lle, uint32_t at)
 {
@@ -1214,14 +1217,15 @@
 	}
 }
 
+template <typename OC, typename SC>
 __global__ void k_tree_emit(uint32_t nS, const uint2 *__restrict__ erec, L0Ranks R, const uint8_t *__restrict__ merged,
 			    const uint2 *__restrict__ dps, const uint32_t *__restrict__ ckey,
 			    const uint32_t *__restrict__ cproc, const uint32_t *__restrict__ voff,
 			    const unsigned long long *__restrict__ start_key, const uint32_t *__restrict__ gid_s,
 			    uint32_t *__restrict__ t_gid, uint8_t *__restrict__ t_flags, uint32_t *__restrict__ t_par,
 			    uint32_t *__restrict__ t_size, uint32_t *__restrict__ t_depth, uint32_t *__restrict__ side_tidx,
-			    uint32_t C, uint32_t *__restrict__ c_ntree, uint32_t *__restrict__ ordcnt, uint32_t *__restrict__ hi0,
-			    uint32_t *__restrict__ mpre, uint32_t *__restrict__ srccnt, uint32_t *__restrict__ sdl,
+			    uint32_t C, uint32_t *__restrict__ c_ntree, OC *__restrict__ ordcnt, uint32_t *__restrict__ hi0,
+			    uint32_t *__restrict__ mpre, SC *__restrict__ srccnt, uint32_t *__restrict__ sdl,
 			    uint32_t *__restrict__ incnt)
 {
 	uint32_t S = BIDX * blockDim.x + threadIdx.x;
@@ -1267,7 +1271,7 @@
 	if (!cproc[c]) {
 		const uint32_t t = tb + 2 * (g - v0);
 		store2_unaligned(t_size + t, 0u, 0u);
-		store2_unaligned(srccnt + t, 0u, 0u);
+		zero2(srccnt + t);
 		store2_unaligned(incnt + t, 0u, 0u);
 		*reinterpret_cast<uint2 *>(side_tidx + 2 * g) = make_uint2(NIL, NIL);
 		return;
@@ -1385,13 +1389,14 @@
 	}
 	return n;
 }
+template <typename OC>
 __global__ void __launch_bounds__(TPB) k_back_edges(uint32_t nS, const uint32_t *__restrict__ loff, const uint32_t *__restrict__ ladj,
 						     const uint2 *__restrict__ dps, const uint32_t *__restrict__ side_tidx,
 						     const uint32_t *__restrict__ ckey, const uint32_t *__restrict__ voff,
 						     const uint32_t *__restrict__ t_par, uint32_t *__restrict__ total_out,
 						     uint32_t *__restrict__ b_src, uint32_t *__restrict__ b_tgt,
 						     uint32_t *__restrict__ b_ord, const uint8_t *__restrict__ dupflag,
-						     uint32_t *__restrict__ ordcnt, uint32_t *__restrict__ hi0, uint32_t *__restrict__ incnt,
+						     OC *__restrict__ ordcnt, uint32_t *__restrict__ hi0, uint32_t *__restrict__ incnt,
 						     uint32_t cap)
 {
 	const uint32_t S0 = BIDX * BE_SIDES + threadIdx.x;
@@ -1406,7 +1411,7 @@
 			uint32_t highest = NIL;
 			k = side_back_edges<false>(S, p, 0, loff, ladj, dps, side_tidx, ckey, voff, t_par, b_src, b_tgt, b_ord, dupflag, incnt, highest,
 						   first2[it][threadIdx.x]);
-			ordcnt[p] = k;
+			ordcnt[p] = (OC)k;
 			hi0[p] = highest;
 			n += k;
 		}
@@ -1770,9 +1775,19 @@
 	tm.end(40);
 
 	tm.begin("tree_emit");
-	LAUNCH(k_tree_emit, std::max(V, C), s, nS, tw.evt, evr, merged, tw.dps, cs.ckey, tw.cproc, cs.voff, start_key, cs.gid_s, sw.t_gid, sw.t_flags,
-	       sw.t_par, sw.t_size, (sw.hairpins || sw.want_depth) ? sw.t_depth : nullptr, tw.side_tidx, C, sw.c_ntree, pw.lsz, pw.hi0, pw.mpre, pw.dlt,
-	       pw.sdl, pw.incnt);
+	auto tree_emit = [&](auto *ordcnt, auto *srccnt) {
+		using OC = std::remove_pointer_t<decltype(ordcnt)>;
+		using SC = std::remove_pointer_t<decltype(srccnt)>;
+		LAUNCH((k_tree_emit<OC, SC>), std::max(V, C), s, nS, tw.evt, evr, merged, tw.dps, cs.ckey, tw.cproc, cs.voff, start_key, cs.gid_s, sw.t_gid,
+		       sw.t_flags, sw.t_par, sw.t_size, (sw.hairpins || sw.want_depth) ? sw.t_depth : nullptr, tw.side_tidx, C, sw.c_ntree, ordcnt,
+		       pw.hi0, pw.mpre, srccnt, pw.sdl, pw.incnt);
+	};
+	if (pw.narrow_ordcnt && pw.narrow_srccnt)
+		tree_emit(pw.ordcnt8, pw.srccnt8);
+	else if (pw.narrow_ordcnt)
+		tree_emit(pw.ordcnt8, pw.dlt);
+	else
+		tree_emit(pw.lsz, pw.dlt);
 	pw.sdl_filled = true;
 	const uint8_t *dupflag = nullptr;
 	if (max_side_links > 64 && E) {
@@ -1789,9 +1804,15 @@
 	}
 	tw.last_dupflag = dupflag;
 	uint32_t *nb0_dev = pw.err + 6;
-	KLAUNCH(k_back_edges, dim3((nS + BE_SIDES - 1) / BE_SIDES), dim3(TPB), 0, s, nS, cs.loff, cs.ladj, tw.dps, tw.side_tidx, cs.ckey,
-		cs.voff, sw.t_par, nb0_dev, pw.b_src, pw.b_tgt, pw.b_ord, dupflag, pw.lsz, pw.hi0, pw.incnt,
-		(uint32_t)std::min<size_t>(pw.nb_cap, 0xFFFFFFFFu));
+	auto back_edges = [&](auto *ordcnt) {
+		KLAUNCH((k_back_edges<std::remove_pointer_t<decltype(ordcnt)>>), dim3((nS + BE_SIDES - 1) / BE_SIDES), dim3(TPB), 0, s, nS, cs.loff, cs.ladj, tw.dps, tw.side_tidx, cs.ckey,
+			cs.voff, sw.t_par, nb0_dev, pw.b_src, pw.b_tgt, pw.b_ord, dupflag, ordcnt, pw.hi0, pw.incnt,
+			(uint32_t)std::min<size_t>(pw.nb_cap, 0xFFFFFFFFu));
+	};
+	if (pw.narrow_ordcnt)
+		back_edges(pw.ordcnt8);
+	else
+		back_edges(pw.lsz);
 	tm.end(6);
 	return NB0_ON_DEVICE;
 }
diff --git a/povu_amd/hip.py b/povu_amd/hip.py
--- a/povu_amd/hip.py
+++ b/povu_amd/hip.py
@@ -18,7 +18,7 @@
     """A device-wide primitive wrote outside its output (raised by its unit-test hook, which guards every output)."""
 
 
-SCAN_SUM, SCAN_MAX, SCAN_U64, SCAN_U8, SCAN_DIFF, SCAN_XOR_PAIR, SCAN_XOR_U128 = range(7)
+SCAN_SUM, SCAN_MAX, SCAN_U64, SCAN_U8, SCAN_DIFF, SCAN_XOR_PAIR, SCAN_XOR_U128, SCAN_DIFF_U8, SCAN_MIXED_PAIR = range(9)
 SCAN_IN_PLACE, SCAN_N_DEV = 0x100, 0x200
 SEG_MIN, SEG_FIRST_LESS, SEG_LAST_LESS = range(3)
 
@@ -267,6 +267,8 @@
     l.povu_hip_debug_tree.restype = C.c_int
     l.povu_hip_debug_tree.argtypes = [C.c_void_p, C.c_uint32, C.POINTER(C.c_uint32), C.c_void_p, C.c_void_p,
                                       C.c_void_p, C.c_void_p]
+    l.povu_hip_last_narrow_counts.restype = C.c_int
+    l.povu_hip_last_narrow_counts.argtypes = [C.c_void_p]
     l.povu_hip_last_black_only_classes.restype = C.c_int
     l.povu_hip_last_black_only_classes.argtypes = [C.c_void_p]
     l.povu_hip_last_crossings.restype = C.c_int
@@ -1077,6 +1079,25 @@
         self._prim_rc(rc, "scan_exclusive_diff_u32")
         return out
 
+    def debug_scan_diff_u8(self, a, sub):
+        a = np.ascontiguousarray(a, dtype=np.uint8)
+        sub = np.ascontiguousarray(sub, dtype=np.uint32)
+        assert a.size == sub.size
+        out = np.empty(a.size, dtype=np.uint32)
+        rc = self._lib.povu_hip_debug_scan(self._ctx, SCAN_DIFF_U8, a.ctypes.data, out.ctypes.data, a.size, sub.ctypes.data,
+                                           None, sub.size)
+        self._prim_rc(rc, "scan_exclusive_diff_u8_u32")
+        return out
+
+    def debug_scan_mixed_pair(self, a, b):
+        a = np.ascontiguousarray(a, dtype=np.uint32)
+        b = np.ascontiguousarray(b, dtype=np.uint8)
+        out, out2 = np.empty_like(a), np.empty(b.size, dtype=np.uint32)
+        rc = self._lib.povu_hip_debug_scan(self._ctx, SCAN_MIXED_PAIR, a.ctypes.data, out.ctypes.data, a.size, b.ctypes.data,
+                                           out2.ctypes.data, b.size)
+        self._prim_rc(rc, "scan_exclusive_u32_u8_pair")
+        return out, out2
+
     def debug_scan_xor_pair(self, a, b):
         a = np.ascontiguousarray(a, dtype=np.uint32)
         b = np.ascontiguousarray(b, dtype=np.uint32)
@@ -1195,6 +1216,9 @@
                                       cls.ctypes.data)
         return dict(gid=gid, typ=typ & 3, black=(typ >> 2) & 1, par=par, cls=cls)
 
+    def last_narrow_counts(self) -> bool:
+        return bool(self._lib.povu_hip_last_narrow_counts(self._ctx))
+
     def last_black_only_classes(self) -> bool:
         return bool(self._lib.povu_hip_last_black_only_classes(self._ctx))
 
```

Result: faster. 3.228 billion (median of 6 runs) (+2.2%).
